# a-rtemis99/hpc_suffix_array

Measured on AMD Instinct MI355X. Metric: suffixes sorted/sec + ms/doubling-round, 1 GiB input at 1/2/4/8 MI355X, higher is better.
Workload: dtype u32

## Files before the change

hpc_suffix_array_amd/_native.py:

```python
from __future__ import annotations

import ctypes
import os
import subprocess

PKG_DIR = os.path.dirname(os.path.abspath(__file__))
LIB_PATH = os.path.join(PKG_DIR, "lib", "libsa_hip.so")
LIB_PATH = os.environ.get("SA_LIB_PATH", LIB_PATH)
CSRC = os.path.join(PKG_DIR, "csrc")

SA_MAX_ROUNDS = 64
KERNEL_KINDS = ["init", "hist_first", "hist_keys", "scan", "scatter_first", "scatter_keys",
                "heads", "heads_scan", "rerank", "seg_count", "seg_scan", "seg_write", "alphabet", "pack",
                "sort_u", "windows", "local_sort", "pivot_keys", "pivot_count", "pivot_write"]
SCHEDULE_PACKED = 0
SCHEDULE_REFERENCE = 1
ROUND1_AUTO = 0
ROUND1_LSD = 1
ROUND1_BUCKETED = 2
SA_K_COUNT = len(KERNEL_KINDS)
FIND_AUTO = 0
FIND_LANE = 1
FIND_WAVE = 2
FIND_LANE_MAX = 3584
FIND_MODES = {"auto": FIND_AUTO, "lane": FIND_LANE, "wave": FIND_WAVE}
BWT_STATS = 258
BWT_TILE = 4096
LOCATE_SA_ORDER = 1
LOCATE_SMALL_CHUNKS = 2
LOCATE_TILE = 2048
LOCATE_ORDERS = {"text": 0, "sa": LOCATE_SA_ORDER}

DROPIN_SYMBOLS = ["create_suffix_array", "destroy_suffix_array", "build_suffix_array",
                  "build_lcp_array", "find_longest_repeated_substring", "is_valid_suffix_array"]
EXT_SYMBOLS = ["sa_context_create", "sa_context_destroy", "sa_context_set_debug", "sa_workspace_bytes", "sa_build_device",
               "sa_build_ex", "sa_check_device", "sa_check", "sa_lcp_device", "sa_lcp", "sa_generate_text_device",
               "sa_alphabet_device", "sa_pack_keys_device", "sa_sort_pairs_device", "sa_scatter_u64_device",
               "sa_gather_u64_device", "sa_running_max_i64_device", "sa_inclusive_sum_i64_device",
               "sa_count_below_u64_device", "sa_select_u8_device",
               "sa_find_device", "sa_find", "sa_find_ex",
               "sa_match_device", "sa_matching_stats_device", "sa_match", "sa_matching_stats",
               "sa_bwt_device", "sa_bwt", "sa_inverse_device", "sa_inverse",
               "sa_locate_device", "sa_locate",
               "sa_dist_begin", "sa_dist_cuts", "sa_dist_plan_cuts", "sa_dist_reserve", "sa_dist_release", "sa_dist_round1", "sa_dist_req_count", "sa_dist_req_fill",
               "sa_dist_answer", "sa_dist_refine",
               "sa_last_error", "sa_host_syncs", "sa_device_count", "sa_version", "sa_struct_size"]


class SAError(RuntimeError):
    """A libsa_hip entry point returned an error code."""


DEBUG_FLAGS = {"no_cmp": 0x1, "no_pk8": 0x2, "no_pad": 0x4, "pad_overflow": 0x8, "no_fast32": 0x10,
               "no_pivot": 0x20, "perm_always": 0x40, "no_xq": 0x80, "xq_overflow": 0x100,
               "no_tied": 0x200, "no_key1_round": 0x400, "no_eonly": 0x800,
               "eonly": 0x1000, "fast32_small": 0x2000, "no_round2_fused": 0x4000,
               "ls_one_wg": 0x8000}


def debug_bits(names) -> int:
    bits = 0
    for x in names or ():
        if x not in DEBUG_FLAGS:
            raise ValueError(f"unknown debug flag {x!r} (one of {sorted(DEBUG_FLAGS)})")
        bits |= DEBUG_FLAGS[x]
    return bits


class SaOpts(ctypes.Structure):
    _fields_ = [("profile", ctypes.c_int32), ("schedule", ctypes.c_int32), ("init_chars", ctypes.c_int32),
                ("radix", ctypes.c_int32), ("round1", ctypes.c_int32), ("debug", ctypes.c_uint32),
                ("span_extra", ctypes.c_int32), ("tune", ctypes.c_int32)]


class SaStats(ctypes.Structure):
    _fields_ = [
        ("rounds", ctypes.c_int32),
        ("n_kinds", ctypes.c_int32),
        ("total_ms", ctypes.c_double),
        ("h2d_ms", ctypes.c_double),
        ("d2h_ms", ctypes.c_double),
        ("round_ms", ctypes.c_double * SA_MAX_ROUNDS),
        ("distinct", ctypes.c_uint64 * SA_MAX_ROUNDS),
        ("passes", ctypes.c_int32 * SA_MAX_ROUNDS),
        ("sorted_n", ctypes.c_uint64 * SA_MAX_ROUNDS),
        ("prefix_len", ctypes.c_uint64 * SA_MAX_ROUNDS),
        ("schedule", ctypes.c_int32),
        ("init_chars", ctypes.c_int32),
        ("sigma", ctypes.c_int32),
        ("sparse_ranks", ctypes.c_int32),
        ("round1", ctypes.c_int32),
        ("largest_window", ctypes.c_int32),
        ("model_bytes", ctypes.c_uint64),
        ("kern_ms", ctypes.c_double * SA_K_COUNT),
        ("kern_launches", ctypes.c_uint64 * SA_K_COUNT),
        ("kern_bytes", ctypes.c_uint64 * SA_K_COUNT),
        ("round1_segments", ctypes.c_int32),
        ("round1_layout", ctypes.c_int32),
        ("round_bytes", ctypes.c_uint64 * SA_MAX_ROUNDS),
        ("round1_windows", ctypes.c_int32 * 4),
    ]

    def to_dict(self) -> dict:
        r = self.rounds
        return {
            "rounds": r,
            "total_ms": self.total_ms,
            "h2d_ms": self.h2d_ms,
            "d2h_ms": self.d2h_ms,
            "round_ms": list(self.round_ms[:r]),
            "distinct": [int(x) for x in self.distinct[:r]],
            "passes": list(self.passes[:r]),
            "sorted_n": [int(x) for x in self.sorted_n[:r]],
            "prefix_len": [int(x) for x in self.prefix_len[:r]],
            "schedule": "reference" if self.schedule == SCHEDULE_REFERENCE else "packed",
            "init_chars": self.init_chars,
            "sigma": self.sigma,
            "sparse_ranks": bool(self.sparse_ranks),
            "round1": {ROUND1_LSD: "lsd", ROUND1_BUCKETED: "bucketed", 3: "pivot"}.get(self.round1, "lsd"),
            "largest_window": self.largest_window,
            "round1_segments": {0: "exact", 1: "padded", 2: "padded-overflow", 3: "striped-records",
                                4: "striped-records-overflow"}.get(self.round1_segments, "exact"),
            "round1_layout": {"compact": bool(self.round1_layout & 1), "pk8": bool(self.round1_layout & 2),
                              "xq": bool(self.round1_layout & 4), "eonly": bool(self.round1_layout & 8)},
            "reference_model_bytes": int(self.model_bytes),
            "round_bytes": [int(x) for x in self.round_bytes[:r]],
            "round1_windows": [int(x) for x in self.round1_windows],
            "kernels": {k: {"ms": self.kern_ms[i], "launches": int(self.kern_launches[i]),
                            "bytes": int(self.kern_bytes[i])} for i, k in enumerate(KERNEL_KINDS)},
        }


DIST_OK = 0
DIST_UNSUPPORTED = 1
DIST_UNBALANCED = 2


class SaDistInfo(ctypes.Structure):
    _fields_ = [("status", ctypes.c_int32), ("sigma", ctypes.c_int32), ("K", ctypes.c_int32),
                ("bucket_bits", ctypes.c_int32), ("m", ctypes.c_uint64), ("sa_off", ctypes.c_uint64),
                ("m_max", ctypes.c_uint64), ("bucket_lo", ctypes.c_uint32), ("bucket_hi", ctypes.c_uint32),
                ("round1_ok", ctypes.c_int32), ("reserved", ctypes.c_int32), ("heads", ctypes.c_uint64),
                ("unsorted", ctypes.c_uint64), ("groups", ctypes.c_uint64)]


class SuffixArrayStruct(ctypes.Structure):
    _fields_ = [("str", ctypes.c_void_p), ("n", ctypes.c_int),
                ("sa", ctypes.POINTER(ctypes.c_int)), ("lcp", ctypes.POINTER(ctypes.c_int))]


_lib = None


def source_hash() -> str:
    import glob
    import hashlib
    h = hashlib.sha256()
    files = sorted(glob.glob(os.path.join(CSRC, "sa_*")) + [os.path.join(CSRC, "Makefile")]
                   + glob.glob(os.path.join(PKG_DIR, "..", "include", "*.h")))
    for p in files:
        with open(p, "rb") as f:
            h.update(os.path.basename(p).encode() + b"\0" + f.read())
    return h.hexdigest()[:16]


def build_library(force: bool = False) -> str:
    if force or not os.path.exists(LIB_PATH):
        subprocess.run(["make", "-s", "-C", CSRC], check=True)
    return LIB_PATH


def lib() -> ctypes.CDLL:
    global _lib
    if _lib is not None:
        return _lib
    if not os.path.exists(LIB_PATH):
        raise SAError(f"{LIB_PATH} is missing: run `make -C {CSRC}` (or __graft_entry__.build())")
    L = ctypes.CDLL(LIB_PATH)
    vp, u64, i32 = ctypes.c_void_p, ctypes.c_uint64, ctypes.c_int
    L.sa_context_create.argtypes = [i32, u64, ctypes.POINTER(vp)]
    L.sa_context_create.restype = i32
    L.sa_context_destroy.argtypes = [vp]
    L.sa_context_destroy.restype = None
    L.sa_context_set_debug.argtypes = [vp, ctypes.POINTER(SaOpts)]
    L.sa_context_set_debug.restype = i32
    L.sa_workspace_bytes.argtypes = [u64]
    L.sa_workspace_bytes.restype = u64
    L.sa_build_device.argtypes = [vp, vp, u64, vp, vp, ctypes.POINTER(SaOpts), ctypes.POINTER(SaStats)]
    L.sa_build_device.restype = i32
    L.sa_build_ex.argtypes = [vp, u64, vp, i32, ctypes.POINTER(SaOpts), ctypes.POINTER(SaStats)]
    L.sa_build_ex.restype = i32
    L.sa_check_device.argtypes = [vp, vp, u64, vp, vp]
    L.sa_check_device.restype = i32
    L.sa_check.argtypes = [vp, u64, vp, i32]
    L.sa_check.restype = i32
    L.sa_lcp_device.argtypes = [vp, vp, u64, vp, vp, ctypes.POINTER(u64), ctypes.POINTER(u64), vp]
    L.sa_lcp_device.restype = i32
    L.sa_lcp.argtypes = [vp, u64, vp, i32, vp, ctypes.POINTER(u64), ctypes.POINTER(u64)]
    L.sa_lcp.restype = i32
    L.sa_alphabet_device.argtypes = [vp, u64, ctypes.POINTER(ctypes.c_uint32), vp]
    L.sa_alphabet_device.restype = i32
    L.sa_pack_keys_device.argtypes = [vp, vp, u64, u64, u64, ctypes.POINTER(ctypes.c_uint16), u64,
                                      ctypes.c_uint32, vp, vp]
    L.sa_pack_keys_device.restype = i32
    L.sa_sort_pairs_device.argtypes = [vp, vp, vp, u64, ctypes.c_uint32, vp, vp, vp]
    L.sa_sort_pairs_device.restype = i32
    L.sa_scatter_u64_device.argtypes = [vp, u64, vp, ctypes.c_int64, vp, u64, vp]
    L.sa_scatter_u64_device.restype = i32
    L.sa_gather_u64_device.argtypes = [vp, vp, u64, vp, ctypes.c_int64, u64, vp]
    L.sa_gather_u64_device.restype = i32
    L.sa_running_max_i64_device.argtypes = [vp, u64, vp]
    L.sa_running_max_i64_device.restype = i32
    L.sa_inclusive_sum_i64_device.argtypes = [vp, u64, vp]
    L.sa_inclusive_sum_i64_device.restype = i32
    L.sa_count_below_u64_device.argtypes = [vp, u64, vp, u64, i32, vp, vp]
    L.sa_count_below_u64_device.restype = i32
    L.sa_select_u8_device.argtypes = [vp, u64, vp, ctypes.POINTER(u64), vp]
    L.sa_select_u8_device.restype = i32
    L.sa_find_device.argtypes = [vp, u64, vp, vp, u64, vp, u64, vp, vp, ctypes.c_uint32, vp]
    L.sa_find_device.restype = i32
    L.sa_find.argtypes = [vp, u64, vp, i32, vp, vp, u64, vp, vp]
    L.sa_find.restype = i32
    L.sa_find_ex.argtypes = [vp, u64, vp, i32, vp, vp, u64, vp, vp, ctypes.c_uint32]
    L.sa_find_ex.restype = i32
    L.sa_match_device.argtypes = [vp, u64, vp, vp, u64, vp, u64, vp, vp, vp, ctypes.c_uint32, vp]
    L.sa_match_device.restype = i32
    L.sa_matching_stats_device.argtypes = [vp, u64, vp, vp, u64, u64, vp, vp, vp, ctypes.c_uint32, vp]
    L.sa_matching_stats_device.restype = i32
    L.sa_match.argtypes = [vp, u64, vp, i32, vp, vp, u64, vp, vp, vp, ctypes.c_uint32]
    L.sa_match.restype = i32
    L.sa_matching_stats.argtypes = [vp, u64, vp, i32, vp, u64, u64, vp, vp, vp, ctypes.c_uint32]
    L.sa_matching_stats.restype = i32
    L.sa_bwt_device.argtypes = [vp, u64, vp, vp, vp, vp]
    L.sa_bwt_device.restype = i32
    L.sa_bwt.argtypes = [vp, u64, vp, i32, vp, vp]
    L.sa_bwt.restype = i32
    L.sa_inverse_device.argtypes = [vp, u64, vp, vp, vp]
    L.sa_inverse_device.restype = i32
    L.sa_inverse.argtypes = [vp, u64, i32, vp]
    L.sa_inverse.restype = i32
    L.sa_locate_device.argtypes = [vp, u64, vp, vp, vp, u64, u64, ctypes.c_uint32, vp, vp, u64, ctypes.POINTER(u64), vp]
    L.sa_locate_device.restype = i32
    L.sa_locate.argtypes = [vp, u64, i32, vp, vp, u64, u64, ctypes.c_uint32, vp, vp, u64]
    L.sa_locate.restype = i32
    DI =ctypes.POINTER(SaDistInfo)
    L.sa_dist_begin.argtypes = [vp, vp, u64, i32, i32, ctypes.POINTER(ctypes.c_uint32), vp, vp, DI]
    L.sa_dist_cuts.argtypes = [vp, ctypes.POINTER(u64), DI]
    L.sa_dist_plan_cuts.argtypes = [i32, u64, i32, ctypes.POINTER(u64), ctypes.POINTER(ctypes.c_uint32),
                                    ctypes.POINTER(u64)]
    L.sa_dist_release.argtypes = [vp]
    L.sa_dist_reserve.argtypes = [vp, u64, i32]
    L.sa_dist_round1.argtypes = [vp, vp, vp, DI, ctypes.POINTER(SaStats)]
    L.sa_dist_req_count.argtypes = [vp, u64, ctypes.POINTER(u64), vp, DI]
    L.sa_dist_req_fill.argtypes = [vp, u64, vp, vp]
    L.sa_dist_answer.argtypes = [vp, vp, u64, vp, vp]
    L.sa_dist_refine.argtypes = [vp, u64, vp, vp, vp, DI]
    for f in (L.sa_dist_begin, L.sa_dist_cuts, L.sa_dist_plan_cuts, L.sa_dist_reserve, L.sa_dist_release,
              L.sa_dist_round1, L.sa_dist_req_count, L.sa_dist_req_fill,
              L.sa_dist_answer, L.sa_dist_refine):
        f.restype = i32
    L.sa_generate_text_device.argtypes = [vp, u64, u64, ctypes.c_char_p, ctypes.c_uint32, vp]
    L.sa_generate_text_device.restype = i32
    L.sa_last_error.argtypes = []
    L.sa_last_error.restype = ctypes.c_char_p
    L.sa_host_syncs.argtypes = []
    L.sa_host_syncs.restype = ctypes.c_uint64
    L.sa_device_count.argtypes = []
    L.sa_device_count.restype = i32
    L.sa_version.argtypes = []
    L.sa_version.restype = ctypes.c_char_p
    P = ctypes.POINTER(SuffixArrayStruct)
    L.create_suffix_array.argtypes = [ctypes.c_char_p, i32]
    L.create_suffix_array.restype = P
    L.destroy_suffix_array.argtypes = [P]
    L.destroy_suffix_array.restype = None
    L.build_suffix_array.argtypes = [P]
    L.build_suffix_array.restype = None
    L.build_lcp_array.argtypes = [P]
    L.build_lcp_array.restype = None
    L.find_longest_repeated_substring.argtypes = [P]
    L.find_longest_repeated_substring.restype = vp
    L.is_valid_suffix_array.argtypes = [P]
    L.is_valid_suffix_array.restype = i32
    _lib = L
    return L


def check(rc: int, what: str) -> int:
    if rc < 0:
        raise SAError(f"{what}: {lib().sa_last_error().decode(errors='replace')} (code {rc})")
    return rc


def device_count() -> int:
    return lib().sa_device_count()


def require_device() -> None:
    if device_count() <= 0:
        raise SAError("no HIP device visible: libsa_hip builds suffix arrays on an MI355X only")
```

hpc_suffix_array_amd/csrc/sa_build.hip:

```cpp
#include <hip/hip_runtime.h>

#include <algorithm>
#include <atomic>
#include <chrono>
#include <cstdarg>
#include <cstdio>
#include <cstdlib>
#include <cstring>
#include <mutex>
#include <string>
#include <thread>
#include <vector>

#include "../../include/sa_hip.h"

#ifndef SA_ALPHA_GRID
#define SA_ALPHA_GRID 2048
#endif

#include "sa_bucket.h"
#include "sa_check.h"
#include "sa_kernels.h"
#include "sa_lcp.h"
#include "sa_limits.h"
// ... 52 lines not shown
#define SA_TRACE(...)                                   \
    do {                                                \
        if (trace_on()) {                               \
            std::fprintf(stderr, "[sa] " __VA_ARGS__);  \
            std::fputc('\n', stderr);                   \
        }                                               \
    } while (0)

#ifndef SA_MAX_CHUNKS
#define SA_MAX_CHUNKS 4096
#endif
constexpr uint32_t kMaxChunks = SA_MAX_CHUNKS;
static_assert(kMaxChunks >= 1 && kMaxChunks <= (1u << 20), "chunk scratch sized for at most 2^20 chunks");
constexpr uint64_t kSparseDiv = 8;
constexpr int kEvPool = 256;
constexpr int kRoundEv = SA_MAX_ROUNDS + 1;
constexpr int kSyncEv = kEvPool + kRoundEv;

static uint64_t align_up(uint64_t x, uint64_t a) { return (x + a - 1) / a * a; }

static uint32_t bit_width(uint64_t x) {
    uint32_t w = 0;
    while (x) { ++w; x >>= 1; }
    return w;
}

static Chunking plan_chunks(uint64_t n) {
    Chunking ch;
    ch.n = n;
    const uint64_t tiles = (n + kTile - 1) / kTile;
    uint64_t tpc = (tiles + kMaxChunks - 1) / kMaxChunks;
    if (tpc == 0) tpc = 1;
    ch.tiles_per_chunk = (uint32_t)tpc;
    ch.chunks = (uint32_t)std::max<uint64_t>(1, (tiles + tpc - 1) / tpc);
    return ch;
}

}

namespace sa { struct DistState; }

struct sa_context {
    int device = 0;
    uint64_t cap = 0;
    uint64_t cap_pad = 0;
    uint64_t ucap = 0;
    uint32_t* rank = nullptr;
    uint64_t* keys[2] = {nullptr, nullptr};
    uint32_t* vals_alt = nullptr;
    uint32_t* vals_u = nullptr;
    uint32_t* u_pos[2] = {nullptr, nullptr};
    uint32_t* u_idx[2] = {nullptr, nullptr};
    uint32_t* u_g[2] = {nullptr, nullptr};
    uint32_t* u_gs[2] = {nullptr, nullptr};
    uint64_t gscap = 0;
    uint64_t* keys_u = nullptr;
    uint64_t kucap = 0;
    uint32_t* segx = nullptr;
    uint64_t segx_words = 0;
    uint32_t* os = nullptr;
    uint32_t* lsd = nullptr;
    uint32_t* lsdx = nullptr;
    uint32_t* segw = nullptr;
    uint64_t* states = nullptr;
    uint32_t epoch = 0;
    int radix = 0;
    int cus = 256;
    uint32_t* member = nullptr;
    uint32_t* hist = nullptr;
    uint32_t* totals = nullptr;
    uint32_t* counts = nullptr;
    uint32_t* words = nullptr;
    uint32_t* alpha = nullptr;
    uint16_t* code = nullptr;
    uint32_t* host_words = nullptr;
    hipEvent_t ev[sa::kEvPool + sa::kRoundEv + 1];
    int ev_ready = 0;
    sa::DistState* dist = nullptr;
    uint32_t dbg = 0;
    int32_t span_extra = 0;
    int32_t tune = 0;
    bool dna = false;
    bool samples_pending = false;
};

namespace sa {

static uint64_t pad_capacity(uint64_t n) { return n + n / 8 + (1ull << 22); }

static uint64_t pad_elems(uint64_t n) {
    const uint64_t m = align_up(std::max<uint64_t>(n, 1), 64);
    return (n >= (1ull << 26) && n <= (1ull << 31)) ? align_up(pad_capacity(n), 64) : m;
}

constexpr uint64_t kMaxRadix = 1024;
static uint64_t tile_states_bytes(uint64_t n) { return ((n + kTile - 1) / kTile + 1) * kMaxRadix * 8; }

static uint64_t ws_bytes(uint64_t n) {
    const uint64_t m = align_up(std::max<uint64_t>(n, 1), 64);
    const uint64_t ku_slack = n >= (1ull << 26) ? n / 16 + 8ull * 1024 * kXqSlack + 64 : 0;
    const uint64_t gs = 2 * (n / 2 + 64) * 4;
    const uint64_t segx = (xq_words(1024) + 1032 + 2ull * kXq * (1ull << 19)) * 4;
    return m * 4 + 2 * m * 8 + m * 4 + (pad_elems(n) - m) * 12 + 7 * m * 4 + (m + ku_slack) * 8 + m / 8 + gs +
           segx + tile_states_bytes(n) + (uint64_t)kRadix * kMaxChunks * 4 + 8192;
}

static void free_ctx_buffers(sa_context* c) {
    hipFree(c->rank);
    hipFree(c->keys[0]);
    hipFree(c->keys[1]);
    hipFree(c->vals_alt);
    hipFree(c->states);
    c->rank = nullptr;
    c->keys[0] = c->keys[1] = nullptr;
    c->vals_alt = nullptr;
    c->states = nullptr;
    c->cap = 0;
    c->cap_pad = 0;
}

static void free_u_buffers(sa_context* c) {
    hipFree(c->vals_u);
    hipFree(c->keys_u);
    hipFree(c->member);
    c->vals_u = nullptr;
    c->keys_u = nullptr;
    c->member = nullptr;
    for (int i = 0; i < 2; ++i) {
        hipFree(c->u_pos[i]);
        hipFree(c->u_idx[i]);
        hipFree(c->u_g[i]);
        hipFree(c->u_gs[i]);
        c->u_pos[i] = c->u_idx[i] = c->u_g[i] = c->u_gs[i] = nullptr;
    }
    c->gscap = 0;
    c->ucap = 0;
    c->kucap = 0;
}

static void set_debug(sa_context* c, const sa_opts* o) {
    c->dbg = o ? o->debug : 0u;
    c->span_extra = o ? o->span_extra : 0;
    c->tune = o ? o->tune : 0;
}

static int ensure_capacity(sa_context* c, uint64_t n) {
    if (n <= c->cap && c->rank) return SA_OK;
    SA_HIP(hipSetDevice(c->device));
    free_ctx_buffers(c);
    const uint64_t m = align_up(std::max<uint64_t>(n, 1), 64);
    const uint64_t mp = pad_elems(n);
    if (hipMalloc(&c->rank, m * 4) != hipSuccess || hipMalloc(&c->keys[0], mp * 8) != hipSuccess ||
        hipMalloc(&c->keys[1], m * 8) != hipSuccess || hipMalloc(&c->vals_alt, mp * 4) != hipSuccess ||
        hipMalloc(&c->states, tile_states_bytes(n)) != hipSuccess ||
        hipMemset(c->states, 0, tile_states_bytes(n)) != hipSuccess) {
        free_ctx_buffers(c);
        (void)hipGetLastError();
        return set_err(SA_E_NOMEM, "device allocation of %.2f GiB workspace failed",
                       (double)ws_bytes(n) / (1ull << 30));
    }
    c->cap = n;
    c->cap_pad = mp;
    SA_TRACE("workspace: rank %p keys0 %p keys1 %p vals_alt %p", (void*)c->rank, (void*)c->keys[0], (void*)c->keys[1],
             (void*)c->vals_alt);
    return SA_OK;
}
// ... 474 lines not shown
            hipLaunchKernelGGL(k_lsd_qbase, dim3(1), dim3(1024), 0, s, (const uint32_t*)qh + p * 8 * kLsdMaxRadix,
                               1u << pl.bits[p], qb);
            tm.end();
            const bool more = p + 1 < pl.P;
            const uint32_t nsh = more ? pl.shift[p + 1] : 0u, nnb = more ? pl.bits[p + 1] : 1u;
            uint32_t* nh = more ? qh + (p + 1) * 8 * kLsdMaxRadix : nullptr;
            uint32_t* tk = qt + p * 8 * 32;
            if (p == 0) {
                tm.begin(SA_K_SCATTER_FIRST);
                SA_TRY(lsd_pass<Src0, PACKED, true>(c, first, n, pl.shift[0], pl.bits[0], qb, tk, kb[0], vb[0], s, nsh,
                                                    nnb, nh, qd, tpq));
                tm.end();
                add_bytes(st, SA_K_SCATTER_FIRST, (8 + pair) * n);
            } else {
                tm.begin(SA_K_SCATTER_KEYS);
                if constexpr (PACKED)
                    SA_TRY(lsd_pass<SrcItems, true, true>(c, SrcItems{kb[(p - 1) & 1]}, n, pl.shift[p], pl.bits[p], qb,
                                                          tk, kb[p & 1], nullptr, s, nsh, nnb, nh, qd, tpq));
                else
                    SA_TRY(lsd_pass<SrcKeys, false, true>(c, SrcKeys{kb[(p - 1) & 1], vb[(p - 1) & 1]}, n, pl.shift[p],
                                                          pl.bits[p], qb, tk, kb[p & 1], vb[p & 1], s, nsh, nnb, nh,
                                                          qd, tpq));
                tm.end();
                add_bytes(st, SA_K_SCATTER_KEYS, 2 * pair * n);
            }
        }
        SA_HIP(hipGetLastError());
        *sorted = kb[(pl.P - 1) & 1];
        return SA_OK;
    }
    tm.begin(SA_K_HIST_FIRST);
    hipLaunchKernelGGL(k_lsd_hist<Src0>, dim3((uint32_t)std::min<uint64_t>((n + 8 * kBlock - 1) / (8 * kBlock),
                                                                           (uint64_t)c->cus * 4)),
                       dim3(kBlock), 0, s, first, n, first_only, lsd_ghist(c));
    tm.end();
    add_bytes(st, SA_K_HIST_FIRST, 8 * n);
    const uint64_t pair = PACKED ? 8 : 12;
    for (uint32_t p = 0; p < pl.P; ++p) {
        uint32_t* base = lsd_base(c) + p * kLsdMaxRadix;
        tm.begin(SA_K_SCAN);
        hipLaunchKernelGGL(k_digit_base_wide, dim3(1), dim3(1024), 0, s,
                           (const uint32_t*)lsd_ghist(c) + p * kLsdMaxRadix, 1u << pl.bits[p], base);
        tm.end();
        const bool more = p + 1 < pl.P;
        const uint32_t nsh = more ? pl.shift[p + 1] : 0u, nnb = more ? pl.bits[p + 1] : 1u;
        uint32_t* nh = more ? lsd_ghist(c) + (p + 1) * kLsdMaxRadix : nullptr;
        if (p == 0) {
            tm.begin(SA_K_SCATTER_FIRST);
            SA_TRY(lsd_pass<Src0, PACKED>(c, first, n, pl.shift[0], pl.bits[0], base, lsd_tickets(c), kb[0], vb[0], s,
                                          nsh, nnb, nh));
            tm.end();
            add_bytes(st, SA_K_SCATTER_FIRST, (8 + pair) * n);
        } else {
            tm.begin(SA_K_SCATTER_KEYS);
            if constexpr (PACKED)
                SA_TRY(lsd_pass<SrcItems, true>(c, SrcItems{kb[(p - 1) & 1]}, n, pl.shift[p], pl.bits[p], base,
                                                lsd_tickets(c) + p, kb[p & 1], nullptr, s, nsh, nnb, nh));
            else
                SA_TRY(lsd_pass<SrcKeys, false>(c, SrcKeys{kb[(p - 1) & 1], vb[(p - 1) & 1]}, n, pl.shift[p],
                                                pl.bits[p], base, lsd_tickets(c) + p, kb[p & 1], vb[p & 1], s, nsh,
                                                nnb, nh));
            tm.end();
            add_bytes(st, SA_K_SCATTER_KEYS, 2 * pair * n);
        }
    }
    SA_HIP(hipGetLastError());
    *sorted = kb[(pl.P - 1) & 1];
    return SA_OK;
}

#ifndef SA_INIT_HIST
#define SA_INIT_HIST 1
#endif
static int build_reference(sa_context* c, const uint8_t* d_text, uint64_t n, uint32_t* d_sa, hipStream_t s,
                           sa_stats* st, Timer& tm) {
    int rc = SA_OK;
    const Chunking ch = plan_chunks(n);
    uint32_t* h_alpha = c->host_words + 64;
    uint16_t* h_code = reinterpret_cast<uint16_t*>(c->host_words + 320);
    SA_HIP(hipMemsetAsync(c->alpha, 0, 8 * 4, s));
    tm.begin(SA_K_ALPHABET);
    {
        const uint32_t grid = (uint32_t)std::min<uint64_t>((n + kBlock * 16 - 1) / (kBlock * 16), SA_ALPHA_GRID);
        hipLaunchKernelGGL(k_alphabet, dim3(grid), dim3(kBlock), 0, s, d_text, n, c->alpha);
    }
    tm.end();
    add_bytes(st, SA_K_ALPHABET, n);
    SA_HIP(hipMemcpyAsync(h_alpha, c->alpha, 8 * 4, hipMemcpyDeviceToHost, s));
    SA_HIP(host_sync(s));
    uint32_t sigma = 0;
    for (int b = 0; b < 256; ++b) h_code[b] = ((h_alpha[b >> 5] >> (b & 31)) & 1u) ? (uint16_t)(++sigma) : 0;
    SA_HIP(hipMemcpyAsync(c->code, h_code, 256 * 2, hipMemcpyHostToDevice, s));
    uint64_t D = sigma;
    const uint64_t perm_min = perm_min_n(c);
    const uint32_t ib = std::max<uint32_t>(1, bit_width(n - 1));
    bool used_perm = false;
    bool hist_ready = false;
    tm.begin(SA_K_INIT);
    {
        const uint32_t w1 = bit_width(D);
        const bool packed1 = c->radix == 0 && 2 * w1 + ib <= 64;
        const LsdPlan pl1 = lsd_plan(2 * w1, packed1 ? ib : 0, lsd_max_bits(c));
        if (SA_INIT_HIST && c->radix == 0 && lsd_xq_ok(c, n, pl1, packed1)) {
            uint32_t tpq;
            uint64_t qspan;
            QDiv qd;
            lsd_xq_span(n, &tpq, &qspan, &qd);
            SA_HIP(hipMemsetAsync(c->lsdx, 0, 8 * kLsdMaxRadix * 4, s));
            const uint64_t grid = std::min<uint64_t>((n + kBlock * 16 - 1) / (kBlock * 16), 4ull * (uint64_t)c->cus);
            hipLaunchKernelGGL(k_init_rank_hist, dim3((uint32_t)grid), dim3(kBlock), 0, s, d_text, n,
                               (const uint16_t*)c->code, c->rank, w1, pl1.shift[0] - (packed1 ? ib : 0u),
                               (1u << pl1.bits[0]) - 1u, qd, c->lsdx);
            hist_ready = true;
        } else {
            const uint64_t grid = std::min<uint64_t>((n + kBlock * 4 - 1) / (kBlock * 4), 4096);
            hipLaunchKernelGGL(k_init_rank_dense, dim3((uint32_t)grid), dim3(kBlock), 0, s, d_text, n,
                               (const uint16_t*)c->code, c->rank);
        }
    }
    tm.end();
    SA_HIP(hipGetLastError());
    add_bytes(st, SA_K_INIT, 5 * n);
    if (st) st->sigma = (int32_t)sigma;

    tm.round_mark();
    for (uint64_t h = 1;; h *= 2) {
        const uint32_t w = bit_width(D);
        const bool packed = c->radix == 0 && 2 * w + ib <= 64;
        SA_TRACE("reference round h=%llu D=%llu w=%u%s", (unsigned long long)h, (unsigned long long)D, w,
                 packed ? " packed" : "");
        SrcRank src{c->rank, n, h, w};
        uint64_t* sorted;
        uint32_t P;
        if (c->radix == 0) {
            const LsdPlan pl = lsd_plan(2 * w, packed ? ib : 0, lsd_max_bits(c));
            P = pl.P;
            rc = packed ? lsd_sort<true>(c, SrcRankPk{c->rank, n, h, w, ib}, n, pl, d_sa, c->vals_alt, s, tm, st,
                                         &sorted, hist_ready)
                        : lsd_sort<false>(c, src, n, pl, d_sa, c->vals_alt, s, tm, st, &sorted, hist_ready);
        } else {
            rc = radix_sort(c, src, 4 * n, ch, 2 * w, d_sa, c->vals_alt, c->keys[0], c->keys[1], s, tm, st, &sorted,
                            &P);
        }
        if (rc) return rc;
        const bool use_perm = packed || n >= perm_min;
        const uint32_t ptiles = (uint32_t)((n + kPermTile - 1) / kPermTile);
        tm.begin(SA_K_HEADS);
        if (use_perm)
            hipLaunchKernelGGL((k_tile_heads<kPermBlock, kPermItems>), dim3(ptiles), dim3(kPermBlock), 0, s,
                               (const uint64_t*)sorted, n, packed ? ib : 0u, perm_tile_off(c));
        else
            hipLaunchKernelGGL(k_heads, dim3(ch.chunks), dim3(kBlock), 0, s, sorted, ch, c->counts, 0u);
        tm.end();
        tm.begin(SA_K_HEADS_SCAN);
        if (use_perm)
            hipLaunchKernelGGL(k_scan_heads, dim3(1), dim3(kBlock), 0, s, perm_tile_off(c), ptiles, c->words);
        else
            hipLaunchKernelGGL(k_scan_heads, dim3(1), dim3(kBlock), 0, s, c->counts, ch.chunks, c->words);
        tm.end();
        SA_HIP(hipGetLastError());
        add_bytes(st, SA_K_HEADS, 8 * n);
        add_bytes(st, SA_K_HEADS_SCAN, 8ull * ch.chunks);
        SA_HIP(hipMemcpyAsync(c->host_words, c->words, 4 * (kPermErrWord + 1), hipMemcpyDeviceToHost, s));
        SA_HIP(host_sync(s));
        if (c->host_words[4]) return set_err(SA_E_INTERNAL, "radix look-back did not complete");
        if (used_perm && c->host_words[kPermErrWord])
            return set_err(SA_E_INTERNAL, "re-rank permutation lost a suffix (flags %u)", c->host_words[kPermErrWord]);
// ... 290 lines not shown
    *sorted = ukb0;
    return SA_OK;
}

static int pivot_round1(sa_context* c, uint64_t n, uint32_t bits1, uint32_t* d_sa, hipStream_t s, Timer& tm,
                        sa_stats* st, bool* done, uint64_t* D, uint64_t* m, uint64_t* G, uint32_t* P) {
    *done = false;
    const Chunking ch = plan_chunks(n);
    const uint64_t* keys = c->keys[1];
    uint32_t* const gs = c->u_pos[1];
    uint32_t* const toff = gs + 2;
    uint32_t* const tid = gs + 4;
    uint32_t* const gP = c->vals_alt;
    uint32_t* const cc = c->hist;
    c->host_words[24] = 0;
    c->host_words[25] = (uint32_t)n;
    SA_HIP(hipMemcpyAsync(gs, c->host_words + 24, 8, hipMemcpyHostToDevice, s));
    tm.begin(SA_K_PIVOT_COUNT);
    hipLaunchKernelGGL((k_pivot_pass<0, true>), dim3(ch.chunks), dim3(kBlock), 0, s, keys, nullptr, nullptr, ch,
                       (const uint32_t*)gs, nullptr, 1u, 0u, cc, gP, nullptr, nullptr, nullptr, nullptr, TiedOut{});
    hipLaunchKernelGGL(k_scan_rows, dim3(3), dim3(kBlock), 0, s, cc, ch.chunks, c->totals);
    tm.end();
    SA_HIP(hipGetLastError());
    add_bytes(st, SA_K_PIVOT_COUNT, 8 * n);
    SA_HIP(hipMemcpyAsync(c->host_words + 16, c->totals, 12, hipMemcpyDeviceToHost, s));
    SA_HIP(host_sync(s));
    const uint64_t t0 = c->host_words[16], t1 = c->host_words[17], t2 = c->host_words[18];
    if (t0 + t1 + t2 != n) return set_err(SA_E_INTERNAL, "round-1 pivot classes %llu + %llu + %llu != %llu",
                                          (unsigned long long)t0, (unsigned long long)t1, (unsigned long long)t2,
                                          (unsigned long long)n);
    SA_TRACE("  round 1: pivot split, tied %llu of %llu", (unsigned long long)t1, (unsigned long long)n);
    if (t1 * 2 < n) return SA_OK;
    const uint64_t mr = t0 + t2;
    uint64_t* const rk = c->keys[0];
    uint32_t* const ridx = c->u_idx[1];
    if (!gs_available(c, n)) return SA_OK;
    tm.begin(SA_K_PIVOT_WRITE);
    hipLaunchKernelGGL(k_pivot_gp, dim3(1), dim3(kBlock), 0, s, (const uint32_t*)gs, 1u, (const uint32_t*)cc, ch,
                       (const uint32_t*)c->totals, gP);
    hipLaunchKernelGGL(k_pivot_tied_scan, dim3(1), dim3(kBlock), 0, s, (const uint32_t*)gP, 1u, toff, tid,
                       c->totals + 4);
    const TiedOut to{nullptr, toff, tid, c->rank, d_sa, c->u_pos[0], c->u_idx[0], c->u_g[0], c->u_gs[0]};
    hipLaunchKernelGGL((k_pivot_pass<3, true>), dim3(ch.chunks), dim3(kBlock), 0, s, keys, nullptr, nullptr, ch,
                       (const uint32_t*)gs, nullptr, 1u, 0u, cc, gP, nullptr, nullptr, rk, ridx, to);
    tm.end();
    SA_HIP(hipGetLastError());
    add_bytes(st, SA_K_PIVOT_WRITE, 8 * n + 16 * t1 + 12 * mr);
    SA_HIP(hipMemcpyAsync(c->host_words + 20, c->totals + 4, 12, hipMemcpyDeviceToHost, s));
    SA_HIP(host_sync(s));
    const uint64_t T = c->host_words[20], Gt = c->host_words[21], Dt = c->host_words[22];
    if (T > t1 || Gt > 1 || Dt > 1)
        return set_err(SA_E_INTERNAL, "round-1 tied block %llu / %llu / %llu out of range", (unsigned long long)T,
                       (unsigned long long)Gt, (unsigned long long)Dt);
    uint32_t Pr = 0;
    uint64_t Dr = 0, mrr = 0, Gr = 0;
    if (mr > 0) {
        const uint32_t Pn = (bits1 + 7) / 8;
        uint32_t* const vfinal = (Pn & 1u) ? c->u_g[1] : ridx;
        uint32_t* const vother = (Pn & 1u) ? ridx : c->u_g[1];
        uint64_t* rs = nullptr;
        int rc = radix_sort(c, SrcKeys{rk, ridx}, 12 * mr, plan_chunks(mr), bits1, vfinal, vother, c->keys_u, rk, s,
                            tm, st, &rs, &Pr);
        if (rc) return rc;
        rc = segments(c, rs, vfinal, plan_chunks(mr), PosGap{t0, t1}, false, nullptr, d_sa, 0, s, tm, st, &Dr, &mrr,
                      &Gr, nullptr, 0, RankMap{}, T, (uint32_t)Gt, c->u_gs[0]);
        if (rc) return rc;
    }
    *done = true;
    *D = Dr + Dt;
    *m = mrr + T;
    *G = Gr + Gt;
    *P = 2 + Pr;
    return SA_OK;
}

static int build_packed(sa_context* c, const uint8_t* d_text, uint64_t n, uint32_t* d_sa, hipStream_t s,
                        const sa_opts* opts, sa_stats* st, Timer& tm) {
    int rc = SA_OK;
    rc = ensure_u_capacity(c, n);
    if (rc) return rc;
    tm.round_mark();
    uint32_t* h_alpha = c->host_words + 64;
    uint16_t* h_code = reinterpret_cast<uint16_t*>(c->host_words + 320);
    SA_HIP(hipMemsetAsync(c->alpha, 0, 8 * 4, s));
    tm.begin(SA_K_ALPHABET);
    {
        const uint32_t grid = (uint32_t)std::min<uint64_t>((n + kBlock * 16 - 1) / (kBlock * 16), SA_ALPHA_GRID);
        hipLaunchKernelGGL(k_alphabet, dim3(grid), dim3(kBlock), 0, s, d_text, n, c->alpha);
    }
    tm.end();
    SA_HIP(hipGetLastError());
    add_bytes(st, SA_K_ALPHABET, n);
    SA_HIP(hipMemcpyAsync(h_alpha, c->alpha, 8 * 4, hipMemcpyDeviceToHost, s));
    const uint32_t tail_n = (uint32_t)std::min<uint64_t>(n, (uint64_t)kMaxK);
    uint8_t* h_tail = reinterpret_cast<uint8_t*>(c->host_words + 2048);
    SA_HIP(hipMemcpyAsync(h_tail, d_text + (n - tail_n), tail_n, hipMemcpyDeviceToHost, s));
    SA_HIP(host_sync(s));
    uint32_t sigma = 0;
    for (int b = 0; b < 256; ++b) h_code[b] = ((h_alpha[b >> 5] >> (b & 31)) & 1u) ? (uint16_t)(++sigma) : 0;
    SA_HIP(hipMemcpyAsync(c->code, h_code, 256 * 2, hipMemcpyHostToDevice, s));
    c->dna = sigma == 4 && h_code['A'] && h_code['C'] && h_code['G'] && h_code['T'];
    uint32_t K = choose_chars(sigma, n, opts ? opts->init_chars : 0);
    const uint64_t base = (uint64_t)sigma + 1;
    const Chunking ch = plan_chunks(n);
    uint64_t* keys1 = nullptr;
    uint32_t ksh1 = 0;
    c->samples_pending = false;
    uint32_t P = 0;

    BucketPlan bp;
    const int r1 = opts ? opts->round1 : SA_ROUND1_AUTO;
    const uint32_t Kb = (opts && opts->init_chars > 0) || sigma <= 1 ? K : min_chars(sigma, n);
    bool bucketed = plan_bucketed(sigma, n, Kb, r1, c->radix, &bp, 1, (c->dbg & SA_DEBUG_NO_CMP) ? 0 : 1);
    if (bucketed && bp.bs.cmp && short_suffix_ties(h_tail, n, tail_n, h_code, sigma, bp.bs.s, bp.bs.R))
        bucketed = plan_bucketed(sigma, n, Kb, r1, c->radix, &bp, 1, 0);
    const bool force_eonly = (c->dbg & SA_DEBUG_EONLY) != 0;
    if (bucketed && bp.bs.cmp == 1 && ((sigma & (sigma - 1)) != 0 || force_eonly) && !(c->dbg & SA_DEBUG_NO_EONLY)) {
        const uint32_t hb = bp.bs.bb - kLoBits;
        BucketPlan b2;
        if ((force_eonly || !plan_pk8(bp, hb, c->dbg, true)) && plan_bucketed(sigma, n, Kb, r1, c->radix, &b2, 1, 2) &&
            (force_eonly || plan_pk8(b2, hb, c->dbg, true)) &&
            !short_suffix_ties(h_tail, n, tail_n, h_code, sigma, b2.bs.s, b2.bs.R, b2.K))
            bp = b2;
    }
    bool fused = false;
    bool r1_pivot = false;
    uint64_t D = 0, m = 0, G = 0;
    uint64_t seg1[3] = {0, 0, 0};
    int r2 = 0;
    if (bucketed) {
        bool done = false;
        rc = round1_bucketed(c, d_text, n, d_sa, bp, full_range(bp, n), s, tm, st, &done, &fused, seg1, &ksh1, true,
                             true, &r2);
        if (rc) return rc;
        bucketed = done;
        if (done) {
            keys1 = c->keys[0];
            P = 2;
            K = bp.K;
        }
    }
    if (!bucketed) {
        const uint32_t bits1 = key_bits(base, K);
        SA_TRACE("packed: sigma=%u K=%u bits=%u", sigma, K, bits1);
        uint64_t top = 1;
        for (uint32_t t = 1; t < K; ++t) top *= base;
        if (c->radix == 0) {
            rc = onesweep_prepare(c, s);
            if (rc) return rc;
        }
        tm.begin(SA_K_PACK);
        hipLaunchKernelGGL(k_pack_text, dim3(ch.chunks), dim3(kBlock), 0, s, d_text, n, (const uint16_t*)c->code, ch,
                           base, top, K, c->keys[1], c->hist, c->radix == 0 ? (bits1 + 7) / 8 : 0u, os_ghist(c));
        tm.end();
        SA_HIP(hipGetLastError());
        add_bytes(st, SA_K_PACK, 9 * n);
        if (c->radix == 0 && !(c->dbg & SA_DEBUG_NO_PIVOT) && n >= (1u << 16)) {
            rc = pivot_round1(c, n, bits1, d_sa, s, tm, st, &r1_pivot, &D, &m, &G, &P);
            if (rc) return rc;
        }
        if (!r1_pivot) {
            SrcKeysIota src{c->keys[1]};
            rc = radix_sort(c, src, 8 * n, ch, bits1, d_sa, c->vals_alt, c->keys[0], c->keys[1], s, tm, st, &keys1,
                            &P, true);
            if (rc) return rc;
        }
    }
    if (st) {
        st->init_chars = (int32_t)K;
        st->sigma = (int32_t)sigma;
        st->round1 = bucketed ? SA_ROUND1_BUCKETED : r1_pivot ? SA_ROUND1_PIVOT : SA_ROUND1_LSD;
    }
    int uo = 0;
    bool sparse = false;
    bool gs_ok[2] = {false, false};
    if (r1_pivot) {
        gs_ok[0] = true;
    } else if (bucketed && fused) {
        D = seg1[0];
        m = seg1[1];
        G = seg1[2];
        sparse = true;
    } else {
        rc = segments(c, keys1, d_sa, ch, PosIdentity{}, true, &sparse, nullptr, uo, s, tm, st, &D, &m, &G, nullptr,
                      0, RankMap{}, 0, 0, gs_buf(c, n, uo));
        if (rc) return rc;
        gs_ok[uo] = gs_buf(c, n, uo) != nullptr;
    }
    uint64_t* ukb0 = keys1 == c->keys[0] ? c->keys[1] : c->keys[0];
    uint64_t* ukb1 = c->keys_u;
    const RankLookup rl{c->rank, c->member, keys1, d_text, (const uint16_t*)c->code, n, base, K,
                        bucketed ? 1u : 0u, bp.bs, bucketed ? c->segw + kBstartOff : nullptr, d_sa, ksh1};
    if (st) st->sparse_ranks = sparse ? 1 : 0;
    auto ensure_samples = [&]() -> int {
        if (!c->samples_pending) return SA_OK;
        c->samples_pending = false;
        const uint64_t ns = (n + (1ull << ksh1) - 1) >> ksh1;
        const uint32_t g = (uint32_t)std::max<uint64_t>(1, std::min<uint64_t>((ns + kBlock - 1) / kBlock, 8192));
        tm.begin(SA_K_SORT_U);
        hipLaunchKernelGGL(k_key1_samples, dim3(g), dim3(kBlock), 0, s, d_text, n, (const uint16_t*)c->code, bp.bs,
                           (const uint32_t*)d_sa, ksh1, keys1);
        tm.end();
        SA_HIP(hipGetLastError());
        add_bytes(st, SA_K_SORT_U, 12 * ns);
        return SA_OK;
    };
    if (r2 == 0) tm.round_mark();
    record_round(st, 0.f, D, P, n, K);
    SA_TRACE("  round 1: D=%llu unsorted=%llu groups=%llu", (unsigned long long)D, (unsigned long long)m,
             (unsigned long long)G);
    if (r2 == 2) {
        tm.round_mark();
        D = n;
        record_round(st, 0.f, D, 1, m, 2 * (uint64_t)K);
        SA_TRACE("  round h=%u: sorted %llu from the local sort's staging, D=%llu", K, (unsigned long long)m,
                 (unsigned long long)D);
        m = 0;
        G = 0;
    }

    const uint32_t wr = bit_width(n);
    for (uint64_t h = K; m > 0; h *= 2) {
        if (h >= 2 * n) return set_err(SA_E_INTERNAL, "doubling did not converge (h=%llu)", (unsigned long long)h);
        const uint32_t wg = G > 1 ? bit_width(G - 1) : 0;
// ... 931 lines not shown
    for (int j = 0; j < kRmItems; ++j) bits |= (b0 + j < m && mask[b0 + j]) ? 1u << j : 0u;
    int64_t o = toff[blockIdx.x] + rm_block_excl<ScanSum>((int64_t)__popc(bits), s_w);
    while (bits) {
        const int j = __builtin_ctz(bits);
        bits &= bits - 1u;
        out[o++] = (int64_t)(b0 + j);
    }
}

template <class Op>
static int scan_i64(int64_t* d_v, uint64_t m, hipStream_t s) {
    const uint64_t tiles = (m + kRmTile - 1) / kRmTile;
    if (tiles > 0xFFFFFFFFull) return set_err(SA_E_INVALID, "m too large");
    int64_t* d_t = nullptr;
    SA_HIP(hipMallocAsync((void**)&d_t, (tiles + 1) * 8, s));
    hipLaunchKernelGGL(k_rmax_tiles<Op>, dim3((uint32_t)tiles), dim3(kRmBlock), 0, s, d_v, m, d_t);
    hipLaunchKernelGGL(k_rmax_carry<Op>, dim3(1), dim3(kRmBlock), 0, s, d_t, tiles);
    hipLaunchKernelGGL(k_rmax_apply<Op>, dim3((uint32_t)tiles), dim3(kRmBlock), 0, s, d_v, m, d_t);
    SA_HIP(hipGetLastError());
    SA_HIP(hipFreeAsync(d_t, s));
    return SA_OK;
}

#include "sa_locate.h"

extern "C" {

int sa_running_max_i64_device(int64_t* d_v, uint64_t m, void* stream) {
    if (m == 0) return SA_OK;
    if (!d_v) return set_err(SA_E_INVALID, "NULL device pointer");
    return scan_i64<ScanMax>(d_v, m, (hipStream_t)stream);
}

int sa_inclusive_sum_i64_device(int64_t* d_v, uint64_t m, void* stream) {
    if (m == 0) return SA_OK;
    if (!d_v) return set_err(SA_E_INVALID, "NULL device pointer");
    return scan_i64<ScanSum>(d_v, m, (hipStream_t)stream);
}

int sa_count_below_u64_device(const uint64_t* d_sorted, uint64_t m, const uint64_t* d_q, uint64_t nq, int right,
                              int64_t* d_out, void* stream) {
    if (nq == 0) return SA_OK;
    if ((!d_sorted && m) || !d_q || !d_out) return set_err(SA_E_INVALID, "NULL device pointer");
    hipStream_t s = (hipStream_t)stream;
    const uint32_t grid = (uint32_t)std::min<uint64_t>((nq + kBlock - 1) / kBlock, 8192);
    if (right) hipLaunchKernelGGL(k_count_below<true>, dim3(grid), dim3(kBlock), 0, s, d_sorted, m, d_q, nq, d_out);
    else hipLaunchKernelGGL(k_count_below<false>, dim3(grid), dim3(kBlock), 0, s, d_sorted, m, d_q, nq, d_out);
    SA_HIP(hipGetLastError());
    return SA_OK;
}

int sa_select_u8_device(const uint8_t* d_mask, uint64_t m, int64_t* d_out, uint64_t* count, void* stream) {
    if (!count) return set_err(SA_E_INVALID, "count is NULL");
    *count = 0;
    if (m == 0) return SA_OK;
    if (!d_mask) return set_err(SA_E_INVALID, "NULL device pointer");
    hipStream_t s = (hipStream_t)stream;
    const uint64_t tiles = (m + kRmTile - 1) / kRmTile;
    if (tiles > 0xFFFFFFFFull) return set_err(SA_E_INVALID, "m too large");
    int64_t* d_t = nullptr;
    int64_t total = 0;
    SA_HIP(hipMallocAsync((void**)&d_t, (tiles + 1) * 8, s));
    hipLaunchKernelGGL(k_sel_count, dim3((uint32_t)tiles), dim3(kRmBlock), 0, s, d_mask, m, d_t);
    hipLaunchKernelGGL(k_rmax_carry<ScanSum>, dim3(1), dim3(kRmBlock), 0, s, d_t, tiles);
    if (d_out) hipLaunchKernelGGL(k_sel_write, dim3((uint32_t)tiles), dim3(kRmBlock), 0, s, d_mask, m, d_t, d_out);
    SA_HIP(hipGetLastError());
    SA_HIP(hipMemcpyAsync(&total, d_t + tiles, 8, hipMemcpyDeviceToHost, s));
    SA_HIP(hipFreeAsync(d_t, s));
    SA_HIP(host_sync(s));
    *count = (uint64_t)total;
    return SA_OK;
}

int sa_alphabet_device(const uint8_t* d_text, uint64_t n, uint32_t present_out[8], void* stream) {
    if (!present_out) return set_err(SA_E_INVALID, "present_out is NULL");
    std::memset(present_out, 0, 32);
    if (n == 0) return SA_OK;
    if (!d_text) return set_err(SA_E_INVALID, "NULL device pointer");
    hipStream_t s = (hipStream_t)stream;
    uint32_t* d_mask = nullptr;
    SA_HIP(hipMallocAsync((void**)&d_mask, 32, s));
    SA_HIP(hipMemsetAsync(d_mask, 0, 32, s));
    const uint32_t grid = (uint32_t)std::min<uint64_t>((n + kBlock * 16 - 1) / (kBlock * 16), 2048);
    hipLaunchKernelGGL(k_alphabet, dim3(grid), dim3(kBlock), 0, s, d_text, n, d_mask);
    SA_HIP(hipGetLastError());
    SA_HIP(hipMemcpyAsync(present_out, d_mask, 32, hipMemcpyDeviceToHost, s));
    SA_HIP(hipFreeAsync(d_mask, s));
    SA_HIP(host_sync(s));
    return SA_OK;
}

int sa_pack_keys_device(sa_context* ctx, const uint8_t* d_text, uint64_t n, uint64_t lo, uint64_t hi,
                        const uint16_t code[256], uint64_t base, uint32_t K, uint64_t* d_keys_out, void* stream) {
    if (lo > hi || hi > n) return set_err(SA_E_INVALID, "bad range [%llu, %llu) of %llu", (unsigned long long)lo,
                                          (unsigned long long)hi, (unsigned long long)n);
    if (K == 0 || K >= (uint32_t)kMaxK || base < 2 || key_bits(base, K) > 64)
        return set_err(SA_E_INVALID, "bad packing K=%u base=%llu", K, (unsigned long long)base);
    if (hi == lo) return SA_OK;
    if (!ctx || !d_text || !d_keys_out || !code) return set_err(SA_E_INVALID, "NULL argument");
    hipStream_t s = (hipStream_t)stream;
    SA_HIP(hipSetDevice(ctx->device));
    uint16_t* h_code = reinterpret_cast<uint16_t*>(ctx->host_words + 320);
    std::memcpy(h_code, code, 512);
    SA_HIP(hipMemcpyAsync(ctx->code, h_code, 512, hipMemcpyHostToDevice, s));
    SA_HIP(host_sync(s));
    uint64_t top = 1;
    for (uint32_t t = 1; t < K; ++t) top *= base;
    const Chunking ch = plan_chunks(hi - lo);
    hipLaunchKernelGGL(k_pack_text, dim3(ch.chunks), dim3(kBlock), 0, s, d_text + lo, n - lo,
                       (const uint16_t*)ctx->code, ch, base, top, K, d_keys_out, (uint32_t*)nullptr, 0u,
                       (uint32_t*)nullptr);
    SA_HIP(hipGetLastError());
    return SA_OK;
}

int sa_sort_pairs_device(sa_context* ctx, const uint64_t* d_keys_in, const uint32_t* d_vals_in, uint64_t m,
                         uint32_t bits, uint64_t* d_keys_out, uint32_t* d_vals_out, void* stream) {
    if (!ctx || !d_keys_in || !d_vals_in || !d_keys_out || !d_vals_out) return set_err(SA_E_INVALID, "NULL argument");
    if (bits == 0 || bits > 64) return set_err(SA_E_INVALID, "bits must be 1..64");
    if (m == 0) return SA_OK;
    if (m > 0xFFFFFFFFull) return set_err(SA_E_INVALID, "m too large");
    if ((const void*)d_keys_in == (const void*)d_keys_out || (const void*)d_vals_in == (const void*)d_vals_out)
        return set_err(SA_E_INVALID, "outputs may not alias inputs");
    hipStream_t s = (hipStream_t)stream;
    SA_HIP(hipSetDevice(ctx->device));
    int rc = ensure_capacity(ctx, m);
    if (rc) return rc;
    ctx->radix = 0;
    SA_HIP(hipMemsetAsync(ctx->words, 0, 64, s));
    Timer tm{ctx, s, false, nullptr};
    const Chunking ch = plan_chunks(m);
    SrcKeys src{d_keys_in, d_vals_in};
    uint64_t* sorted;
    uint32_t P;
    rc = radix_sort(ctx, src, 12 * m, ch, bits, d_vals_out, ctx->vals_alt, d_keys_out, ctx->keys[1], s, tm, nullptr,
                    &sorted, &P);
    if (rc) return rc;
    if (sorted != d_keys_out) SA_HIP(hipMemcpyAsync(d_keys_out, sorted, m * 8, hipMemcpyDeviceToDevice, s));
    SA_HIP(hipMemcpyAsync(ctx->host_words, ctx->words, 20, hipMemcpyDeviceToHost, s));
    SA_HIP(host_sync(s));
    if (ctx->host_words[4]) return set_err(SA_E_INTERNAL, "radix look-back did not complete");
    return SA_OK;
}

int sa_generate_text_device(uint8_t* d_out, uint64_t n, uint64_t seed, const uint8_t* alphabet, uint32_t sigma,
                            void* stream) {
    if (n == 0) return SA_OK;
    if (!d_out || !alphabet || sigma == 0 || sigma > 256) return set_err(SA_E_INVALID, "bad generator arguments");
    Alphabet a;
    std::memset(a.sym, 0, sizeof a.sym);
    std::memcpy(a.sym, alphabet, sigma);
    const uint32_t grid = (uint32_t)std::min<uint64_t>((n + kBlock - 1) / kBlock, 16384);
    hipLaunchKernelGGL(k_gen_text, dim3(grid), dim3(kBlock), 0, (hipStream_t)stream, d_out, n, seed, a, sigma);
    SA_HIP(hipGetLastError());
    return SA_OK;
}

int sa_dist_begin(sa_context* ctx, const uint8_t* d_text, uint64_t n, int world, int rank,
                  const uint32_t present[8], uint64_t* d_coarse, void* stream, sa_dist_info* info) {
    if (!ctx || !info) return set_err(SA_E_INVALID, "NULL argument");
    return dist_begin(ctx, d_text, n, world, rank, present, d_coarse, (hipStream_t)stream, info);
}

int sa_dist_cuts(sa_context* ctx, const uint64_t* h_coarse, sa_dist_info* info) {
    if (!ctx || !info) return set_err(SA_E_INVALID, "NULL argument");
    return dist_cuts(ctx, h_coarse, info);
}
// ... 92 lines not shown
```

hpc_suffix_array_amd/csrc/sa_dropin.cpp:

```cpp
#include <cstddef>
#include <cstdint>
#include <cstdio>
#include <cstdlib>
#include <cstring>
#include <vector>

#include "../../include/sa_hip.h"
#include "../../include/suffix_array.h"

static_assert(sizeof(SuffixArray) == 32, "SuffixArray must keep the reference's 32-byte layout");
static_assert(offsetof(SuffixArray, n) == 8 && offsetof(SuffixArray, sa) == 16 && offsetof(SuffixArray, lcp) == 24,
              "SuffixArray field offsets must match suffix_array.h:16-21");

[[noreturn]] static void die(const char* what) {
    std::fprintf(stderr, "libsa_hip: %s failed: %s\n", what, sa_last_error());
    std::abort();
}

extern "C" {

SuffixArray* create_suffix_array(const char* S, int n) {
    if (n < 0) return nullptr;
    SuffixArray* sa = (SuffixArray*)std::malloc(sizeof(SuffixArray));
    if (!sa) return nullptr;
    sa->n = n;
    sa->str = (char*)std::malloc((size_t)n + 1);
    if (!sa->str) {
        std::free(sa);
        return nullptr;
    }
    std::strncpy(sa->str, S ? S : "", (size_t)n);
    sa->str[n] = '\0';
    sa->sa = (int*)std::malloc((size_t)(n ? n : 1) * sizeof(int));
    sa->lcp = (int*)std::malloc((size_t)(n ? n : 1) * sizeof(int));
    if (!sa->sa || !sa->lcp) {
        std::free(sa->str);
        std::free(sa->sa);
        std::free(sa->lcp);
        std::free(sa);
        return nullptr;
    }
    return sa;
}

void destroy_suffix_array(SuffixArray* sa) {
    if (!sa) return;
    std::free(sa->str);
    std::free(sa->sa);
    std::free(sa->lcp);
    std::free(sa);
}

void build_suffix_array(SuffixArray* sa) {
    if (!sa || sa->n <= 0) return;
    if (sa_build_ex((const uint8_t*)sa->str, (uint64_t)sa->n, sa->sa, 4, nullptr, nullptr) != SA_OK)
        die("build_suffix_array");
}

void build_lcp_array(SuffixArray* sa) {
    if (!sa || sa->n <= 0) return;
    if (sa_lcp((const uint8_t*)sa->str, (uint64_t)sa->n, sa->sa, 4, sa->lcp, nullptr, nullptr) != SA_OK)
        die("build_lcp_array");
}

char* find_longest_repeated_substring(SuffixArray* sa) {
    if (!sa || !sa->lcp) return nullptr;
    int best = 0, at = -1;
    for (int r = 1; r < sa->n; ++r)
        if (sa->lcp[r] > best) {
            best = sa->lcp[r];
            at = r;
        }
    if (best == 0) return nullptr;
    char* out = (char*)std::malloc((size_t)best + 1);
    if (!out) return nullptr;
    std::strncpy(out, sa->str + sa->sa[at], (size_t)best);
    out[best] = '\0';
    return out;
}

int is_valid_suffix_array(SuffixArray* sa) {
    if (!sa || sa->n <= 0) return 1;
    const int r = sa_check((const uint8_t*)sa->str, (uint64_t)sa->n, sa->sa, 4);
    if (r < 0) die("is_valid_suffix_array");
    return r;
}

}

extern "C" uint64_t sa_struct_size(int which) {
    return which == 0 ? sizeof(sa_stats) : which == 1 ? sizeof(sa_opts) : 0;
}
```

hpc_suffix_array_amd/csrc/sa_kernels.h:

```cpp
#pragma once
#include <hip/hip_runtime.h>
#include <stdint.h>

#include "sa_search.h"

namespace sa {

constexpr int kWave = 64;
constexpr int kBlock = 256;
constexpr int kWaves = kBlock / kWave;
constexpr int kItems = 16;
constexpr int kTile = kBlock * kItems;
constexpr int kWaveTile = kWave * kItems;
constexpr int kRadix = 256;

__device__ __forceinline__ uint32_t lane_id() { return threadIdx.x & (kWave - 1); }
__device__ __forceinline__ uint32_t wave_id() { return threadIdx.x / kWave; }
__device__ __forceinline__ uint64_t lanemask_lt() { return (1ull << lane_id()) - 1ull; }

struct SrcRank {
    const uint32_t* __restrict__ rank;
    uint64_t n;
    uint64_t h;
    uint32_t w;
    __device__ __forceinline__ uint64_t key(uint64_t e) const {
        const uint64_t r0 = rank[e];
        const uint64_t r1 = (e + h < n) ? rank[e + h] : 0u;
        return (r0 << w) | r1;
    }
    __device__ __forceinline__ uint32_t val(uint64_t e) const { return (uint32_t)e; }
    static constexpr bool kRaw = true;
    __device__ __forceinline__ uint64_t raw(uint64_t e) const {
        return (uint64_t)rank[e] | ((uint64_t)((e + h < n) ? rank[e + h] : 0u) << 32);
    }
    __device__ __forceinline__ uint64_t finish(uint64_t r, uint64_t) const {
        return ((r & 0xFFFFFFFFull) << w) | (r >> 32);
    }
};

struct SrcText {
    const uint8_t* __restrict__ text;
    const uint16_t* __restrict__ code;
    uint64_t n;
    uint64_t base;
    uint32_t K;
    __device__ __forceinline__ uint64_t key(uint64_t e) const {
        uint64_t x = 0;
        if (e + K <= n) {
            for (uint32_t t = 0; t < K; ++t) x = x * base + code[text[e + t]];
        } else {
            for (uint32_t t = 0; t < K; ++t) x = x * base + ((e + t < n) ? code[text[e + t]] : 0u);
        }
        return x;
    }
    __device__ __forceinline__ uint32_t val(uint64_t e) const { return (uint32_t)e; }
};

struct BucketSpec {
    uint64_t pow_s1;
    uint64_t powR1;
    uint64_t cmul;
    uint32_t sigma, s, R, rb;
    uint32_t bb, bsh;
    uint32_t cmp;
};

__host__ __device__ __forceinline__ uint64_t bucket_low(const BucketSpec& b, uint64_t r, uint64_t L) {
    if (b.cmp == 2) return r;
    if (b.cmp) return 2 * r + (L >= b.s + b.R ? 1u : 0u);
    if (L < b.s) return L - 1;
    const uint64_t tl = L - b.s < b.R ? L - b.s : b.R;
    return b.s + r * (b.R + 1) + tl;
}

struct CodeMap {
    const uint16_t* __restrict__ code;
    __device__ __forceinline__ uint32_t operator[](uint32_t b) const {
        const uint32_t c = code[b];
        return c ? c - 1u : 0u;
    }
};

constexpr int kKeyWords = 8;

template <bool FULL, class Map>
__device__ __forceinline__ uint64_t key1_words(const uint8_t* __restrict__ text, uint64_t n, const Map& s_map,
// ... 494 lines not shown
            bool ok;
            const uint64_t m = wave_heads(keys, w0 + (uint64_t)j * kWave, e1, prev_last, key, ok, kshift);
            cnt += (uint32_t)__popcll(m);
        }
    }
    uint32_t tot;
    block_exclusive_sum(lane_id() == 0 ? cnt : 0u, s_tmp, &tot);
    if (threadIdx.x == 0) counts[c] = tot;
}

__global__ __launch_bounds__(kBlock) void k_scan_heads(uint32_t* __restrict__ counts, uint32_t chunks,
                                                       uint32_t* __restrict__ d_total) {
    __shared__ uint32_t s_tmp[kWaves];
    uint32_t carry = 0;
    for (uint32_t base = 0; base < chunks; base += kBlock * 4) {
        uint32_t v[4], sum = 0;
#pragma unroll
        for (int j = 0; j < 4; ++j) {
            const uint32_t i = base + threadIdx.x * 4 + j;
            v[j] = (i < chunks) ? counts[i] : 0u;
            sum += v[j];
        }
        uint32_t tot;
        uint32_t off = block_exclusive_sum(sum, s_tmp, &tot) + carry;
#pragma unroll
        for (int j = 0; j < 4; ++j) {
            const uint32_t i = base + threadIdx.x * 4 + j;
            if (i < chunks) counts[i] = off;
            off += v[j];
        }
        carry += tot;
    }
    if (threadIdx.x == 0) *d_total = carry;
}

__global__ __launch_bounds__(kBlock) void k_rerank(const uint64_t* __restrict__ keys,
                                                   const uint32_t* __restrict__ idx, Chunking ch,
                                                   const uint32_t* __restrict__ chunk_off,
                                                   uint32_t* __restrict__ rank) {
    __shared__ uint32_t s_wtot[kWaves];
    __shared__ uint32_t s_tmp[kWaves];
    const uint32_t c = blockIdx.x;
    const uint64_t e0 = ch.begin(c), e1 = ch.end(c);
    uint32_t run = chunk_off[c];
    for (uint64_t tb = e0; tb < e1; tb += kTile) {
        const uint64_t w0 = tb + (uint64_t)wave_id() * kWaveTile;
        uint64_t prev_last = (w0 > 0 && w0 < e1) ? keys[w0 - 1] : 0ull;
        uint64_t m[kItems];
        uint32_t wsum = 0;
#pragma unroll
        for (int j = 0; j < kItems; ++j) {
            uint64_t key;
            bool ok;
            m[j] = wave_heads(keys, w0 + (uint64_t)j * kWave, e1, prev_last, key, ok);
            wsum += (uint32_t)__popcll(m[j]);
        }
        if (lane_id() == 0) s_wtot[wave_id()] = wsum;
        __syncthreads();
        uint32_t woff = run, ttot = 0;
#pragma unroll
        for (int w = 0; w < kWaves; ++w) {
            const uint32_t x = s_wtot[w];
            woff += (w < (int)wave_id()) ? x : 0u;
            ttot += x;
        }
        __syncthreads();
        const uint64_t le_mask = lanemask_lt() | (1ull << lane_id());
#pragma unroll
        for (int j = 0; j < kItems; ++j) {
            const uint64_t e = w0 + (uint64_t)j * kWave + lane_id();
            if (e < e1) {
                const uint32_t x = idx[e];
                if (x < ch.n) rank[x] = woff + (uint32_t)__popcll(m[j] & le_mask);
            }
            woff += (uint32_t)__popcll(m[j]);
        }
        run += ttot;
    }
    (void)s_tmp;
}


__global__ __launch_bounds__(kBlock) void k_alphabet(const uint8_t* __restrict__ text, uint64_t n,
                                                     uint32_t* __restrict__ present) {
    __shared__ uint32_t s_m[kBlock * 9];
    uint32_t* m = s_m + threadIdx.x * 9;
#pragma unroll
    for (int i = 0; i < 8; ++i) m[i] = 0;
    auto add = [&](uint32_t b) { atomicOr(&m[b >> 5], 1u << (b & 31u)); };
    const uint64_t stride = (uint64_t)gridDim.x * kBlock * 16;
    auto whole = [&](uint64_t i) { return i + 16 <= n && (((uintptr_t)(text + i)) & 15) == 0; };
    uint64_t i = ((uint64_t)blockIdx.x * kBlock + threadIdx.x) * 16;
    uint4 v = make_uint4(0u, 0u, 0u, 0u);
    if (i < n && whole(i)) v = *reinterpret_cast<const uint4*>(text + i);
    uint32_t step = 0;
    for (; i < n; i += stride) {
        if (step && (step & (step - 1)) == 0) {
            uint32_t all = ~0u;
#pragma unroll
            for (int q = 0; q < 8; ++q) {
                uint32_t x = m[q];
#pragma unroll
                for (int o = 32; o >= 1; o >>= 1) x |= __shfl_xor(x, o, kWave);
                all &= x;
            }
            if (all == ~0u) break;
        }
        ++step;
        const uint64_t in = i + stride;
        uint4 vn = make_uint4(0u, 0u, 0u, 0u);
        if (in < n && whole(in)) vn = *reinterpret_cast<const uint4*>(text + in);
        if (whole(i)) {
            const uint32_t w4[4] = {v.x, v.y, v.z, v.w};
            uint32_t o = v.x | v.y | v.z | v.w, a = v.x & v.y & v.z & v.w;
            o |= o >> 16;
            o |= o >> 8;
            a &= a >> 16;
            a &= a >> 8;
            if (((o ^ a) & 0xE0u) == 0u) {
                uint32_t bits = 0;
#pragma unroll
                for (int q = 0; q < 4; ++q)
#pragma unroll
                    for (int b = 0; b < 4; ++b) bits |= 1u << ((w4[q] >> (8 * b)) & 31u);
                atomicOr(&m[(o & 0xFFu) >> 5], bits);
            } else {
#pragma unroll
                for (int q = 0; q < 4; ++q)
#pragma unroll
                    for (int b = 0; b < 4; ++b) add((w4[q] >> (8 * b)) & 0xFFu);
            }
        } else {
            for (uint64_t j = i; j < n && j < i + 16; ++j) add(text[j]);
        }
        v = vn;
    }
    __shared__ uint32_t s_or[8];
    if (threadIdx.x < 8) s_or[threadIdx.x] = 0;
    __syncthreads();
#pragma unroll
    for (int i = 0; i < 8; ++i) {
        uint32_t x = m[i];
#pragma unroll
        for (int o = 32; o >= 1; o >>= 1) x |= __shfl_xor(x, o, kWave);
        if (lane_id() == 0 && x) atomicOr(&s_or[i], x);
    }
    __syncthreads();
    if (threadIdx.x < 8) {
        const uint32_t x = s_or[threadIdx.x];
        if (x & ~__hip_atomic_load(&present[threadIdx.x], __ATOMIC_RELAXED, __HIP_MEMORY_SCOPE_AGENT))
            atomicOr(&present[threadIdx.x], x);
    }
}

__device__ __forceinline__ void hist_add_runs_valid(uint32_t (*s_h)[kRadix], uint64_t k, bool valid, uint32_t p_lo,
                                                    uint32_t p_hi, uint32_t row0) {
    const uint32_t lane = lane_id();
    const uint64_t above = lane == 63 ? 0ull : (~0ull << (lane + 1));
    for (uint32_t p = p_lo; p < p_hi; ++p) {
        const uint32_t d = valid ? ((uint32_t)(k >> (8 * p)) & 0xFFu) : 0x100u;
        const uint32_t dl = __shfl_up(d, 1, 64);
        const bool head = lane == 0 || dl != d;
        const uint64_t hm = __ballot(head) & above;
        const uint32_t next = hm ? (uint32_t)__ffsll((long long)hm) - 1u : 64u;
        if (head && valid) atomicAdd(&s_h[row0 + p][d], next - lane);
    }
}

constexpr int kPackRun = kTile / kBlock;
constexpr int kMaxK = 64;
constexpr int kPackMaxPasses = 8;

__global__ __launch_bounds__(kBlock) void k_pack_text(const uint8_t* __restrict__ text, uint64_t avail,
                                                      const uint16_t* __restrict__ code, Chunking ch,
                                                      uint64_t base, uint64_t top, uint32_t K,
                                                      uint64_t* __restrict__ keys, uint32_t* __restrict__ hist,
                                                      uint32_t passes, uint32_t* __restrict__ ghist) {
    __shared__ uint16_t s_code[256];
    __shared__ uint16_t s_c[kTile + kMaxK];
    __shared__ uint32_t s_hist[kPackMaxPasses][kRadix];
    __shared__ uint64_t s_k[kTile + kTile / kPackRun];
    s_code[threadIdx.x] = code[threadIdx.x];
    for (int i = threadIdx.x; i < kPackMaxPasses * kRadix; i += kBlock) (&s_hist[0][0])[i] = 0;
    const uint32_t c = blockIdx.x;
    const uint64_t e0 = ch.begin(c), e1 = ch.end(c);
    const uint64_t n = avail;
    auto count = [&](uint64_t key, bool valid) {
        if (passes == 0) hist_add_runs_valid(s_hist, key, valid, 0, 1, wave_id());
        else hist_add_runs_valid(s_hist, key, valid, 0, passes, 0);
    };
    __syncthreads();
    for (uint64_t tb = e0; tb < e1; tb += kTile) {
        {
            const uint64_t i = tb + (uint64_t)threadIdx.x * 16;
            uint16_t* dst = s_c + threadIdx.x * 16;
            if (i + 16 <= n && (((uintptr_t)(text + i)) & 15) == 0) {
                const uint4 v = *reinterpret_cast<const uint4*>(text + i);
                const uint32_t w4[4] = {v.x, v.y, v.z, v.w};
#pragma unroll
                for (int q = 0; q < 4; ++q)
#pragma unroll
                    for (int b = 0; b < 4; ++b) dst[4 * q + b] = s_code[(w4[q] >> (8 * b)) & 0xFFu];
            } else {
                for (int q = 0; q < 16; ++q) dst[q] = (i + q < n) ? s_code[text[i + q]] : (uint16_t)0;
            }
            if (threadIdx.x < K) {
                const uint64_t h = tb + kTile + threadIdx.x;
                s_c[kTile + threadIdx.x] = (h < n) ? s_code[text[h]] : (uint16_t)0;
            }
        }
        __syncthreads();
        const uint32_t l0 = threadIdx.x * kPackRun;
        uint64_t x = 0;
        for (uint32_t t = 0; t < K; ++t) x = x * base + s_c[l0 + t];
        uint64_t* kd = s_k + threadIdx.x * (kPackRun + 1);
        kd[0] = x;
        count(x, tb + l0 < e1);
#pragma unroll
        for (int j = 1; j < kPackRun; ++j) {
            x = (x - (uint64_t)s_c[l0 + j - 1] * top) * base + s_c[l0 + j - 1 + K];
            kd[j] = x;
            count(x, tb + l0 + j < e1);
        }
        __syncthreads();
#pragma unroll
        for (int j = 0; j < kPackRun; ++j) {
            const uint32_t q = j * kBlock + threadIdx.x;
            const uint64_t g = tb + q;
            if (g < e1) keys[g] = s_k[q + q / kPackRun];
        }
        __syncthreads();
    }
    if (passes == 0) {
        uint32_t s = 0;
#pragma unroll
        for (int w = 0; w < kWaves; ++w) s += s_hist[w][threadIdx.x];
        if (hist) hist[(uint64_t)threadIdx.x * ch.chunks + c] = s;
    } else {
        for (uint32_t p = 0; p < passes; ++p) {
            const uint32_t v = s_hist[p][threadIdx.x];
            if (v) atomicAdd(&ghist[p * kRadix + threadIdx.x], v);
        }
    }
}

struct PosIdentity {
    __device__ __forceinline__ uint32_t operator()(uint64_t s) const { return (uint32_t)s; }
};
struct PosArray {
    const uint32_t* __restrict__ p;
    __device__ __forceinline__ uint32_t operator()(uint64_t s) const { return p[s]; }
};
struct PosGap {
// ... 290 lines not shown
```

hpc_suffix_array_amd/csrc/sa_limits.h:

```cpp
#pragma once
#include <cstdint>

namespace sa {

constexpr uint32_t kXqQueues = 8;
constexpr uint32_t kXqRegionSlack = 2048;
constexpr uint32_t kXqMaxDigits = 1024;

constexpr uint64_t xq_region_space(uint64_t m) {
    return m + m / 16 + (uint64_t)kXqQueues * kXqMaxDigits * kXqRegionSlack;
}

constexpr bool xq_offsets_fit(uint64_t m) { return xq_region_space(m) <= 0xFFFFFFFFull; }

}
```

hpc_suffix_array_amd/csrc/sa_round1.h:

```cpp
#pragma once

#ifndef SA_HIST_WPC
#define SA_HIST_WPC 64
#endif
#ifndef SA_REC_STRIPED
#define SA_REC_STRIPED 1
#endif
#ifndef SA_BB_EXTRA
#define SA_BB_EXTRA 0
#endif
#ifndef SA_ITEMS_A
#define SA_ITEMS_A 12
#endif
#ifndef SA_TEXT_BLOCK
#define SA_TEXT_BLOCK 512
#endif
#ifndef SA_LIST_BLOCK
#define SA_LIST_BLOCK 1024
#endif


#ifndef SA_SEG_BLOCK
#define SA_SEG_BLOCK 1024
#endif
#ifndef SA_SEG_XQ
#define SA_SEG_XQ 1
#endif
#ifndef SA_ITEMS_B
#define SA_ITEMS_B 10
#endif
#ifndef SA_ITEMS_PK
#define SA_ITEMS_PK 12
#endif
#ifndef SA_KEY_SAMPLE
#define SA_KEY_SAMPLE 4
#endif
constexpr uint32_t kKeySample = SA_KEY_SAMPLE;
#ifndef SA_LAZY_SAMPLES
#define SA_LAZY_SAMPLES 1
#endif
constexpr uint64_t kPadMinN = 1ull << 26;
#ifndef SA_LS_VARIANT
#define SA_LS_VARIANT 0
#endif
static int ls_variant(const sa_context* c) {
    const uint32_t t = ((uint32_t)c->tune >> 16) & 0xFu;
    return t ? (int)(t - 1u) : SA_LS_VARIANT;
}

static uint32_t text_stripes(const sa_context* c) {
    const uint32_t e = ((uint32_t)c->tune >> 8) & 0xFFu;
    const uint32_t v = e ? e : 8u;
    return v >= 8 ? 8u : v >= 4 ? 4u : v >= 2 ? 2u : 1u;
}

__global__ __launch_bounds__(kLoRadix) void k_sum_rows(const uint32_t* __restrict__ in, uint32_t rows,
                                                       uint32_t* __restrict__ out) {
    uint32_t t = 0;
    for (uint32_t r = 0; r < rows; ++r) t += in[r * kLoRadix + threadIdx.x];
    out[threadIdx.x] = t;
}
constexpr uint64_t kPadMaxN = 1ull << 31;
constexpr int kUsFlagWord = 12;

static uint32_t key1_bits(const BucketSpec& bs) {
    unsigned __int128 dmax = 1;
    for (uint32_t t = 0; t < bs.s; ++t) dmax *= bs.sigma;
    const unsigned __int128 kmax = ((dmax - 1) << bs.rb) | (((unsigned __int128)1 << bs.rb) - 1);
    uint32_t kw = 0;
    for (unsigned __int128 x = kmax + 1; x; x >>= 1) ++kw;
    return kw;
}
constexpr uint32_t kPadStartOff = kLoRadix + 1024;
constexpr uint32_t kPadDenseOff = kPadStartOff + kLoRadix + 64;

struct BucketPlan {
    BucketSpec bs{};
    uint32_t ib = 0;
    uint32_t K = 0;
};

static bool plan_bucketed(uint32_t sigma, uint64_t n, uint32_t K, int round1, int radix, BucketPlan* p,
                          int world = 1, int cmp = 0) {
    if (round1 == SA_ROUND1_LSD || radix != 0 || sigma < 2 || n < 2) return false;
    if (round1 == SA_ROUND1_AUTO && n < kBucketMinN) return false;
    uint32_t bb = std::max<uint32_t>(16u, bit_width(n - 1) > 13 ? bit_width(n - 1) - 13 : 0u);
    if (world <= 1) bb = std::min<uint32_t>(bb, 18u);
    bb += SA_BB_EXTRA;
    if (bb > 18 + (uint32_t)bit_width((uint64_t)std::max(world, 1) - 1) || bb > 24) return false;
    uint64_t ps = 1;
    uint32_t s = 0;
    while (ps < (1ull << bb)) {
        ps *= sigma;
        ++s;
    }
    while (ps % (1ull << bb) != 0 && ps < (64ull << bb) && s + 1 < K && ps * sigma <= (1ull << 32)) {
        ps *= sigma;
        ++s;
    }
    if (ps > (1ull << 32)) return false;
    if (K <= s || K > (uint32_t)kMaxK) return false;
    const uint32_t ib = bit_width(n - 1);
    const uint32_t bd = bit_width(ps - 1);
    const uint32_t span = bit_width((ps + (1ull << bb) - 1) >> bb) + 1;
    for (uint32_t R = K - s; R >= 1; --R) {
        unsigned __int128 pr = 1;
        for (uint32_t t = 0; t < R; ++t) pr *= sigma;
        unsigned __int128 lowmax = cmp == 2 ? pr - 1 : cmp ? 2 * pr - 1 : s + (pr - 1) * (R + 1) + R;
        uint32_t rb = 0;
        while (lowmax) {
            ++rb;
            lowmax >>= 1;
        }
        if (bd + rb > 64 || rb + span + ib > 64) continue;
        p->bs.pow_s1 = ps / sigma;
        p->bs.powR1 = (uint64_t)(pr / sigma);
        p->bs.cmul = (1ull << 48) / ps;
        p->bs.bb = bb;
        p->bs.bsh = 48u - bb;
        p->bs.sigma = sigma;
        p->bs.s = s;
        p->bs.R = R;
        p->bs.rb = rb;
        p->bs.cmp = (uint32_t)cmp;
        p->ib = ib;
        p->K = s + R;
        return true;
    }
    return false;
}

static bool short_suffix_ties(const uint8_t* tail, uint64_t n, uint32_t t, const uint16_t* code, uint32_t sigma,
                              uint32_t s, uint32_t R, uint32_t last = 0) {
    auto dig = [&](uint8_t x) -> uint32_t { return code[x] ? code[x] - 1u : 0u; };
    const uint32_t K = s + R;
    if (last == 0) last = K - 1;
    uint64_t Ds[kMaxK + 1];
    unsigned __int128 rs[kMaxK + 1];
    uint32_t cnt = 0;
    for (uint32_t L = 1; L <= last && L <= n && L <= t; ++L) {
        const uint8_t* x = tail + (t - L);
        uint64_t D = 0;
        unsigned __int128 r = 0;
        for (uint32_t q = 0; q < s; ++q) D = D * sigma + (q < L ? dig(x[q]) : 0u);
        for (uint32_t q = s; q < K; ++q) r = r * sigma + (q < L ? dig(x[q]) : 0u);
        for (uint32_t o = 0; o < cnt; ++o)
            if (Ds[o] == D && rs[o] == r) return true;
        Ds[cnt] = D;
        rs[cnt] = r;
        ++cnt;
    }
    return false;
}

static bool plan_pk8(const BucketPlan& bp, uint32_t hb, uint32_t dbg, bool np2 = false) {
    const uint32_t sg = bp.bs.sigma;
    if (sg < 2 || (dbg & SA_DEBUG_NO_PK8)) return false;
    if ((sg & (sg - 1)) != 0) {
        if (!np2) return false;
        const uint64_t ps = bp.bs.pow_s1 * sg;
        const uint64_t per = ((ps + (1ull << bp.bs.bb) - 1) >> bp.bs.bb) + 1;
        return hb + bit_width(per - 1) + bp.bs.rb + bp.ib <= 64;
    }
    const uint32_t lg = (uint32_t)__builtin_ctz(sg);
    if (lg * bp.bs.s < bp.bs.bb) return false;
    return hb + (lg * bp.bs.s - bp.bs.bb) + bp.bs.rb + bp.ib <= 64;
}

struct BucketRange {
    uint32_t blo = 0, bhi = 0;
    uint64_t m = 0;
    uint64_t sa_off = 0;
    bool always_u = false;
    uint32_t* rank = nullptr;
    uint32_t* member = nullptr;
    uint32_t* prefix = nullptr;
    uint32_t* tmp_rank = nullptr;
};

static BucketRange full_range(const BucketPlan& bp, uint64_t n) {
    BucketRange r;
    r.blo = 0;
    r.bhi = 1u << bp.bs.bb;
    r.m = n;
    return r;
}

static uint32_t range_hb(uint32_t nb) {
    const uint32_t w = bit_width(nb > 1 ? nb - 1 : 1);
    return std::max<uint32_t>(7u, w > kLoBits ? w - kLoBits : 0u);
}

static int round1_bucketed(sa_context* c, const uint8_t* d_text, uint64_t n, uint32_t* d_sa, const BucketPlan& bp,
                           const BucketRange& br_, hipStream_t s, Timer& tm, sa_stats* st, bool* done, bool* fused,
                           uint64_t seg[3], uint32_t* ksh, bool allow_pad = true, bool allow_xq = true,
                           int* round2 = nullptr) {
    *done = false;
    *fused = false;
    *ksh = 0;
    if (round2) *round2 = 0;
    const uint64_t m = br_.m;
    const uint32_t blo = br_.blo, bhi = br_.bhi;
    if (bhi <= blo || bhi - blo > (1u << 18)) return set_err(SA_E_INTERNAL, "bucket range [%u, %u)", blo, bhi);
    int rc = onesweep_prepare(c, s);
    if (rc) return rc;
    SA_HIP(hipMemsetAsync(c->words, 0, 12, s));
    SA_HIP(hipMemsetAsync(c->words + 5, 0, 28, s));
    const bool listed = m * 10 <= n * 3;
    uint64_t* const lkeys = c->keys_u;
    uint32_t* const lpos = c->vals_u;
    const uint64_t rtiles = (n + kTile - 1) / kTile;
    const uint32_t rgrid = (uint32_t)(std::min<uint64_t>(rtiles, (uint64_t)SA_HIST_WPC * (uint32_t)c->cus) /
                                      kRecStripes * kRecStripes);
    const uint64_t rcap64 = (c->dbg & SA_DEBUG_PAD_OVERFLOW) ? m / kRecStripes / 2 + 1
                                                             : (m + m / 8) / kRecStripes + 2 * (uint64_t)kTile;
    const bool striped = SA_REC_STRIPED && listed && allow_pad && !(c->dbg & SA_DEBUG_NO_PAD) &&
                         rtiles >= 4ull * kRecStripes && rgrid >= kRecStripes && kRecStripes * rcap64 <= c->ucap;
    const uint32_t rcap = (uint32_t)std::min<uint64_t>(rcap64, UINT32_MAX);
    uint32_t* const rcur = c->hist;
    const bool padded = allow_pad && !listed && blo == 0 && bhi == (1u << bp.bs.bb) && n >= kPadMinN &&
                        n <= kPadMaxN && c->cap_pad >= pad_capacity(n) && !(c->dbg & SA_DEBUG_NO_PAD);
    const uint32_t ssh = std::max<uint32_t>(6u, bit_width(n) > 21 ? bit_width(n) - 21 : 0u);
    uint32_t* const pstart = os_base(c) + kPadStartOff;
    uint32_t* const dlo = os_base(c) + kPadDenseOff;
    if (st) st->round1_segments = padded ? 1 : striped ? 3 : 0;
    tm.begin(SA_K_PACK);
    if (padded) {
        const bool pow2 = (bp.bs.sigma & (bp.bs.sigma - 1)) == 0;
        const uint32_t g = (uint32_t)std::max<uint64_t>(1, std::min<uint64_t>(((n >> ssh) + kBlock - 1) / kBlock,
                                                                               4u * (uint32_t)c->cus));
        if (pow2)
            hipLaunchKernelGGL(k_bucket_sample<true>, dim3(g), dim3(kBlock), 0, s, d_text, n,
                               (const uint16_t*)c->code, bp.bs, ssh, os_ghist(c));
        else
            hipLaunchKernelGGL(k_bucket_sample<false>, dim3(g), dim3(kBlock), 0, s, d_text, n,
                               (const uint16_t*)c->code, bp.bs, ssh, os_ghist(c));
        hipLaunchKernelGGL(k_pad_starts, dim3(1), dim3(kLoRadix), 0, s, (const uint32_t*)os_ghist(c), ssh,
                           (c->dbg & SA_DEBUG_PAD_OVERFLOW) ? 1u : 0u, (uint32_t)c->cap_pad, pstart);
    } else {
        const uint64_t tiles = (n + kTile - 1) / kTile;
        const uint32_t g = (uint32_t)std::max<uint64_t>(1, std::min<uint64_t>(tiles, (uint64_t)SA_HIST_WPC * (uint32_t)c->cus));
        const bool pow2 = (bp.bs.sigma & (bp.bs.sigma - 1)) == 0;
        uint32_t* const wgcnt = c->hist;
        uint32_t* const wgoff = c->hist + g;
#define SA_HIST_G(G, P, L, W)                                                                                 \
    hipLaunchKernelGGL((k_bucket_hist<P, false, L>), dim3(G), dim3(kBlock), 0, s, d_text, n,                  \
                       (const uint16_t*)c->code, bp.bs, os_ghist(c), 0ull, n, blo, bhi, lkeys, lpos, W, rcap,  \
                       c->words + 11)
#define SA_HIST_ID_G(G, L, W)                                                                                 \
    hipLaunchKernelGGL((k_bucket_hist<true, false, L, true>), dim3(G), dim3(kBlock), 0, s, d_text, n,         \
                       (const uint16_t*)c->code, bp.bs, os_ghist(c), 0ull, n, blo, bhi, lkeys, lpos, W, rcap,  \
                       c->words + 11)
#define SA_HIST(P, L, W) SA_HIST_G(g, P, L, W)
#define SA_HIST_ID(L, W) SA_HIST_ID_G(g, L, W)
        const bool ident = bp.bs.sigma == 256;
        if (striped) {
            SA_HIP(hipMemsetAsync(rcur, 0, kRecStripes * kRecCurStride * 4, s));
            if (ident) SA_HIST_ID_G(rgrid, 3, rcur);
            else if (pow2 && SA_DNA_SWAR && c->dna)
                hipLaunchKernelGGL((k_bucket_hist<true, false, 3, false, true>), dim3(rgrid), dim3(kBlock), 0, s, d_text,
                                   n, (const uint16_t*)c->code, bp.bs, os_ghist(c), 0ull, n, blo, bhi, lkeys, lpos, rcur,
                                   rcap, c->words + 11);
            else if (pow2) SA_HIST_G(rgrid, true, 3, rcur);
            else SA_HIST_G(rgrid, false, 3, rcur);
            SA_HIP(hipMemcpyAsync(c->host_words + 11, c->words + 11, 4, hipMemcpyDeviceToHost, s));
            SA_HIP(host_sync(s));
            if (c->host_words[11]) {
                SA_TRACE("  bucketed round 1: a record stripe overflowed, again with the counting scan");
                tm.end();
                const int rc = round1_bucketed(c, d_text, n, d_sa, bp, br_, s, tm, st, done, fused, seg, ksh, false,
                                               allow_xq, round2);
                if (st) st->round1_segments = 4;
                return rc;
            }
        } else if (ident && listed) SA_HIST_ID(1, wgcnt);
        else if (pow2 && listed) SA_HIST(true, 1, wgcnt);
        else if (pow2) SA_HIST(true, 0, wgcnt);
        else if (listed) SA_HIST(false, 1, wgcnt);
        else SA_HIST(false, 0, wgcnt);
        if (listed && !striped) {
            hipLaunchKernelGGL(k_exscan_u32, dim3(1), dim3(kBlock), 0, s, (const uint32_t*)wgcnt, wgoff, g);
            if (ident) SA_HIST_ID(2, wgoff);
            else if (pow2) SA_HIST(true, 2, wgoff);
            else SA_HIST(false, 2, wgoff);
        }
#undef SA_HIST
#undef SA_HIST_ID
#undef SA_HIST_G
#undef SA_HIST_ID_G
    }
    tm.end();
    add_bytes(st, SA_K_PACK, padded ? (n >> ssh) * 64 : n + (striped ? 12 * m : listed ? n + 12 * m : 0));
    const uint32_t hb = (blo == 0 && bhi == (1u << bp.bs.bb)) ? bp.bs.bb - kLoBits : range_hb(bhi - blo);
    if (hb < 7 || hb > 10) return set_err(SA_E_INTERNAL, "second bucket pass of %u bits", hb);
    const uint32_t nb_tab = 1u << (hb + kLoBits);
    const bool np2 = (bp.bs.sigma & (bp.bs.sigma - 1)) != 0;
    const bool pk8 = plan_pk8(bp, hb, c->dbg, !br_.always_u);
    uint32_t bits1 = 0;
    if (bp.bs.cmp) {
        const uint64_t ps = bp.bs.pow_s1 * bp.bs.sigma, per = (ps + (1ull << bp.bs.bb) - 1) >> bp.bs.bb;
        const bool exact = (ps & ((1ull << bp.bs.bb) - 1)) == 0;
        bits1 = bit_width(exact ? per - 1 : per) + bp.bs.rb;
        if (c->span_extra > 0) bits1 = std::min<uint32_t>(bits1 + (uint32_t)c->span_extra, 64u - bp.ib);
    }
    const bool fast32 = bits1 > (uint32_t)kSubBits && bits1 - kSubBits <= kLowMax &&
                        (m / (uint64_t)(bhi - blo) >= 4ull * kWinStride || (c->dbg & SA_DEBUG_FAST32_SMALL)) &&
                        !(c->dbg & SA_DEBUG_NO_FAST32);
    static_assert(kXqQueues == kXq && kXqRegionSlack == kXqSlack, "sa_limits.h mirrors sa_split.h");
    const bool xq = SA_SEG_XQ && allow_xq && fast32 && c->cus % (int)kXq == 0 && !(c->dbg & SA_DEBUG_NO_XQ) &&
                    c->kucap >= xq_region_space(m) + kWave && xq_offsets_fit(m);
    if (st) st->round1_layout = (bp.bs.cmp ? 1 : 0) | (pk8 ? 2 : 0) | (xq ? 4 : 0) | (bp.bs.cmp == 2 ? 8 : 0);
    const uint64_t xqw = xq_words(1u << hb);
    uint32_t* xq_dh = nullptr;
    uint32_t* xq_pc = nullptr;
    uint32_t* xq_pn = nullptr;
    if (xq) {
        const uint64_t need = xqw + 1032 + 2ull * kXq * nb_tab;
        if (c->segx_words < need) {
            hipFree(c->segx);
            c->segx = nullptr;
            c->segx_words = 0;
            if (hipMalloc(&c->segx, need * 4) != hipSuccess) {
                (void)hipGetLastError();
                return set_err(SA_E_NOMEM, "second-pass queue workspace (%llu words)", (unsigned long long)need);
            }
            c->segx_words = need;
        }
        xq_dh = c->segx + xqw;
        xq_pc = xq_dh + 1032;
        xq_pn = xq_pc + (uint64_t)kXq * nb_tab;
    }
    uint32_t* const g_lo = os_ghist(c);
    uint32_t* const g_hi = os_ghist(c) + kLoRadix;
    const uint32_t stripes = padded ? text_stripes(c) : 1u;
    uint32_t* const cursor = stripes > 1 ? c->hist : os_ghist(c) + 5 * kRadix;
    uint32_t* const cursor_sum = stripes > 1 ? c->hist + kMaxStripes * kLoRadix : cursor;
    if (stripes > 1) SA_HIP(hipMemsetAsync(cursor, 0, (size_t)stripes * kLoRadix * 4, s));
    if (!padded) {
        tm.begin(SA_K_SCAN);
        hipLaunchKernelGGL(k_digit_base_wide, dim3(1), dim3(1024), 0, s, (const uint32_t*)g_lo, kLoRadix, os_base(c));
        tm.end();
    }
    tm.begin(SA_K_SCATTER_FIRST);
    {
        constexpr int kItemsA = SA_ITEMS_A;
        constexpr int kTextBlock = SA_TEXT_BLOCK;
        const bool pow2 = (bp.bs.sigma & (bp.bs.sigma - 1)) == 0;
        const bool dna = SA_DNA_SWAR && c->dna && bp.bs.s + bp.bs.R + kItemsA - 1 <= 32 && 2 * bp.bs.s <= 32;
        const bool ident = SA_TEXT_IDENT && bp.bs.sigma == 256 && bp.bs.s + bp.bs.R <= 8 && bp.bs.s <= 4;
        auto text_grid = [&](int block) {
            const uint64_t tile = (uint64_t)block * kItemsA;
            return (uint32_t)std::max<uint64_t>(
                1, std::min<uint64_t>((n + tile - 1) / tile, (uint64_t)c->cus * (kSpBlock / block)));
        };
#define SA_TEXT_PASS(P, PK, BLK, DNA, ID)                                                                     \
    hipLaunchKernelGGL((k_split_text<kItemsA, BLK, P, PK, DNA, ID>), dim3(text_grid(BLK)), dim3(BLK), 0, s, d_text, n, \
                       (const uint16_t*)c->code, bp.bs, (const uint32_t*)(padded ? pstart : os_base(c)),           \
                       os_tickets(c), c->keys[0], c->vals_alt, g_hi, cursor, m, blo, bhi,                          \
                       padded ? (const uint32_t*)pstart + 1 : nullptr, padded ? c->words + 11 : nullptr, hb, bp.ib, \
                       stripes)
        if (listed) {
            constexpr int kItemsL = SA_ITEMS_B, kListBlock = SA_LIST_BLOCK;
            const uint64_t tl = (uint64_t)kListBlock * kItemsL;
            const uint32_t gl = (uint32_t)std::max<uint64_t>(
                1, std::min<uint64_t>((m + tl - 1) / tl, (uint64_t)c->cus * (kSpBlock / kListBlock)));
            if (pk8)
                hipLaunchKernelGGL((k_split_list<kItemsL, kListBlock, true>), dim3(gl), dim3(kListBlock), 0, s, bp.bs,
                                   (const uint64_t*)lkeys, (const uint32_t*)lpos, m, blo, (const uint32_t*)os_base(c),
                                   os_tickets(c), c->keys[0], c->vals_alt, g_hi, cursor, hb, bp.ib,
                                   striped ? (const uint32_t*)rcur : nullptr, rcap);
            else
                hipLaunchKernelGGL((k_split_list<kItemsL, kListBlock, false>), dim3(gl), dim3(kListBlock), 0, s, bp.bs,
                                   (const uint64_t*)lkeys, (const uint32_t*)lpos, m, blo, (const uint32_t*)os_base(c),
                                   os_tickets(c), c->keys[0], c->vals_alt, g_hi, cursor, 0u, 0u,
                                   striped ? (const uint32_t*)rcur : nullptr, rcap);
        } else if (pk8 && np2) {
#define SA_TEXT_NP2(R32)                                                                                         \
    hipLaunchKernelGGL((k_split_text<kItemsA, kSpBlock, false, true, false, false, R32>), dim3(text_grid(kSpBlock)), \
                       dim3(kSpBlock), 0, s, d_text, n, (const uint16_t*)c->code, bp.bs,                           \
                       (const uint32_t*)(padded ? pstart : os_base(c)), os_tickets(c), c->keys[0], c->vals_alt, g_hi, \
                       cursor, m, blo, bhi, padded ? (const uint32_t*)pstart + 1 : nullptr,                        \
                       padded ? c->words + 11 : nullptr, hb, bp.ib, stripes)
            if (bp.bs.powR1 * (uint64_t)bp.bs.sigma <= 0xFFFFFFFFull && !(((uint32_t)c->tune >> 28) & 1u))
                SA_TEXT_NP2(true);
            else
                SA_TEXT_NP2(false);
#undef SA_TEXT_NP2
        } else if (pk8 && dna) {
            SA_TEXT_PASS(true, true, kTextBlock, true, false);
        } else if (pk8 && ident) {
            SA_TEXT_PASS(true, true, kTextBlock, false, true);
        } else if (pk8) {
            SA_TEXT_PASS(true, true, kTextBlock, false, false);
        } else if (pow2 && ident) {
            SA_TEXT_PASS(true, false, kTextBlock, false, true);
        } else if (pow2) {
            SA_TEXT_PASS(true, false, kTextBlock, false, false);
        } else if (bp.bs.powR1 * (uint64_t)bp.bs.sigma <= 0xFFFFFFFFull && !(((uint32_t)c->tune >> 28) & 1u)) {
            hipLaunchKernelGGL((k_split_text<kItemsA, kSpBlock, false, false, false, false, true>),
                               dim3(text_grid(kSpBlock)), dim3(kSpBlock), 0, s, d_text, n, (const uint16_t*)c->code,
                               bp.bs, (const uint32_t*)(padded ? pstart : os_base(c)), os_tickets(c), c->keys[0],
                               c->vals_alt, g_hi, cursor, m, blo, bhi, padded ? (const uint32_t*)pstart + 1 : nullptr,
                               padded ? c->words + 11 : nullptr, hb, bp.ib, stripes);
        } else {
            SA_TEXT_PASS(false, false, kSpBlock, false, false);
        }
#undef SA_TEXT_PASS
    }
    tm.end();
    add_bytes(st, SA_K_SCATTER_FIRST, listed ? (pk8 ? 20 : 24) * m : n + (pk8 ? 8 : 12) * m);
    tm.begin(SA_K_SCAN);
    hipLaunchKernelGGL(k_digit_base_wide, dim3(1), dim3(1024), 0, s, (const uint32_t*)g_hi, 1u << hb,
                       os_base(c) + kLoRadix);
    if (xq)
        hipLaunchKernelGGL(k_xq_dh, dim3(1), dim3(1024), 0, s, (const uint32_t*)g_hi, 1u << hb,
                           (c->dbg & SA_DEBUG_XQ_OVERFLOW) ? 1u : 0u, xq_dh);
    if (padded) {
        if (stripes > 1)
            hipLaunchKernelGGL(k_sum_rows, dim3(1), dim3(kLoRadix), 0, s, (const uint32_t*)cursor, stripes, cursor_sum);
        hipLaunchKernelGGL(k_digit_base_wide, dim3(1), dim3(1024), 0, s, (const uint32_t*)cursor_sum, kLoRadix, dlo);
    }
    tm.end();
    tm.begin(SA_K_SCATTER_KEYS);
    {
        constexpr int kItemsB = SA_ITEMS_B, kItemsPk = SA_ITEMS_PK;
        const SrcBucketKeys sb{c->keys[0], c->vals_alt, bp.bs.rb, bp.bs.bsh, bp.bs.cmul, blo};
        const SrcPk8 sp{c->keys[0]};
        uint32_t* tk = os_tickets(c) + 1;
        const uint32_t* hbase = os_base(c) + kLoRadix;
        SA_HIP(hipMemsetAsync(c->segw, 0, segw_words(1u << hb) * 4, s));
        SegXq sx;
        if (xq) {
            SA_HIP(hipMemsetAsync(c->segx, 0, xqw * 4, s));
            sx.cur = c->segx;
            sx.sbase = reinterpret_cast<uint64_t*>(c->segx + (uint64_t)kXq * kSegs * (1u << hb));
            sx.done = c->segx + 3ull * kXq * kSegs * (1u << hb);
            sx.tickets = sx.done + kXq * kSegs;
            sx.dh = xq_dh;
            sx.err2 = c->words + 9;
            sx.cap = (uint32_t)std::min<uint64_t>(c->kucap, UINT32_MAX);
        }
        constexpr int kSegBlock = SA_SEG_BLOCK;
        const int sblk = hb <= 9 ? kSegBlock : kSpBlock;
        const uint64_t ut = (uint64_t)sblk * (pk8 ? kItemsPk : kItemsB);
        const uint64_t units = (m + ut - 1) / ut + kSegs;
        const uint32_t grid = xq ? (uint32_t)c->cus * (kSpBlock / sblk)
                                 : (uint32_t)std::max<uint64_t>(1, std::min<uint64_t>(units, (uint64_t)c->cus * (kSpBlock / sblk)));
        switch (hb) {
#define SA_SEG_LAUNCH(S, B, SRC, SH, IT)                                                                      \
    if (xq)                                                                                                   \
        hipLaunchKernelGGL((k_split_seg<S, B, IT, (B <= 9 ? kSegBlock : kSpBlock), true>), dim3(grid),        \
                           dim3(B <= 9 ? kSegBlock : kSpBlock), 0, s, SRC, m, SH,                              \
                           (const uint32_t*)(padded ? pstart : os_base(c)), hbase, c->segw, tk, bp.ib, c->keys_u,      \
                           c->words + 4, padded ? (const uint32_t*)cursor : nullptr,                           \
                           padded ? (const uint32_t*)dlo : nullptr, stripes, sx);                              \
    else                                                                                                      \
        hipLaunchKernelGGL((k_split_seg<S, B, IT, (B <= 9 ? kSegBlock : kSpBlock)>), dim3(grid),                \
                           dim3(B <= 9 ? kSegBlock : kSpBlock), 0, s, SRC, m, SH,                              \
                           (const uint32_t*)(padded ? pstart : os_base(c)), hbase, c->segw, tk, bp.ib, c->keys_u,      \
                           c->words + 4, padded ? (const uint32_t*)cursor : nullptr,                           \
                           padded ? (const uint32_t*)dlo : nullptr, stripes)
#define SA_SEG_PASS(B)                                                                                        \
    case B:                                                                                                   \
        if (pk8) SA_SEG_LAUNCH(SrcPk8, B, sp, 64u - B, kItemsPk);                                             \
        else SA_SEG_LAUNCH(SrcBucketKeys, B, sb, kLoBits, kItemsB);                                           \
        break;
            SA_SEG_PASS(7)
            SA_SEG_PASS(8)
            SA_SEG_PASS(9)
            SA_SEG_PASS(10)
#undef SA_SEG_PASS
#undef SA_SEG_LAUNCH
            default: return set_err(SA_E_INTERNAL, "second bucket pass of %u bits", hb);
        }
        const uint32_t gb = (uint32_t)std::min<uint64_t>(((uint64_t)nb_tab + kBlock) / kBlock, 1024);
        uint32_t* bstart = c->segw + kBstartOff;
        uint32_t* bdmin = bstart + kBstartWords;
#define SA_BSTARTS(R)                                                                                         \
    if (xq)                                                                                                   \
        hipLaunchKernelGGL(k_bucket_starts_xq<R>, dim3(R), dim3(kLoRadix), 0, s, hbase, (const uint32_t*)sx.cur, \
                           (const uint32_t*)xq_dh, m, bp.bs.cmul, bp.bs.bsh, bstart, bdmin, xq_pc, xq_pn, blo); \
    else                                                                                                      \
        hipLaunchKernelGGL(k_bucket_starts<R>, dim3(gb), dim3(kBlock), 0, s, (const uint32_t*)(padded ? dlo : os_base(c)), \
                           hbase, (const uint32_t*)c->segw, m, bp.bs.cmul, bp.bs.bsh, bstart, bdmin, blo)
        switch (hb) {
            case 7: SA_BSTARTS(128); break;
            case 8: SA_BSTARTS(256); break;
            case 9: SA_BSTARTS(512); break;
            default: SA_BSTARTS(1024); break;
        }
#undef SA_BSTARTS
    }
    tm.end();
    add_bytes(st, SA_K_SCATTER_KEYS, (pk8 ? 16 : 20) * m);
    SA_HIP(hipGetLastError());
    const uint64_t nw = (m + kWinStride - 1) / kWinStride;
    uint32_t* ws = c->vals_alt;
    uint32_t* list = c->vals_alt + nw + 1;
    tm.begin(SA_K_WINDOWS);
    {
        const uint32_t g1 = (uint32_t)std::min<uint64_t>((nw + kBlock) / kBlock, 8192);
        hipLaunchKernelGGL(k_window_starts_tab, dim3(g1), dim3(kBlock), 0, s, (const uint32_t*)(c->segw + kBstartOff),
                           nb_tab, m, nw, ws, list + 4 * nw + 2);
        const uint32_t g2 = (uint32_t)std::min<uint64_t>((nw + kBlock - 1) / kBlock, 1024);
        hipLaunchKernelGGL(k_window_list, dim3(g2), dim3(kBlock), 0, s, (const uint32_t*)ws, nw, list, c->words);
    }
    tm.end();
    add_bytes(st, SA_K_WINDOWS, 8 * nw);
    SA_HIP(hipGetLastError());
    SA_HIP(hipMemcpyAsync(c->host_words, c->words, 48, hipMemcpyDeviceToHost, s));
    uint32_t* skew = list + nw;
    uint32_t* cnt_u = skew + nw;
    uint32_t* cnt_g = cnt_u + nw + 1;
    uint32_t* const rank_arr = br_.rank ? br_.rank : c->rank;
    uint32_t* const member = br_.member ? br_.member : c->member;
    SA_HIP(hipEventRecord(c->ev[kSyncEv], s));
    SA_HIP(hipMemsetAsync(cnt_u, 0, (2 * nw + 2) * 4, s));
    SA_HIP(hipMemsetAsync(member, 0, (n + 31) / 32 * 4, s));
    SA_HIP(host_sync_event(c->ev[kSyncEv]));
    if (c->host_words[4]) return set_err(SA_E_INTERNAL, "radix look-back did not complete");
    if (padded && c->host_words[11]) {
        SA_TRACE("  bucketed round 1: padded segment overflow, again with exact digit totals");
        const int rc = round1_bucketed(c, d_text, n, d_sa, bp, br_, s, tm, st, done, fused, seg, ksh, false, allow_xq,
                                       round2);
        if (st) st->round1_segments = 2;
        return rc;
    }
    if (xq && c->host_words[9]) {
        SA_TRACE("  bucketed round 1: second-pass queue overflow, again with one region");
        return round1_bucketed(c, d_text, n, d_sa, bp, br_, s, tm, st, done, fused, seg, ksh, allow_pad, false,
                               round2);
    }
    if (st) st->largest_window = (int32_t)std::min<uint32_t>(c->host_words[5], INT32_MAX);
    if (c->host_words[5] > (uint32_t)kBsCap) {
        SA_TRACE("  bucketed round 1: window of %u > %d suffixes, full sort instead", c->host_words[5], kBsCap);
        return SA_OK;
    }
    BucketRel br{cnt_g + nw + 1, c->segw + kBstartOff, c->segw + kBstartOff + kBstartWords, bp.bs.rb};
    br.bits1 = bits1;
    SegOut so{rank_arr, member, br_.sa_off, c->u_pos[1], c->u_idx[1], c->u_g[1], cnt_u, cnt_g, kKeySample};
    so.tmp_rank = br_.prefix ? br_.tmp_rank : nullptr;
    so.samples = (SA_LAZY_SAMPLES && !br_.always_u && !(c->dbg & SA_DEBUG_NO_KEY1_ROUND)) ? 0u : 1u;
    uint32_t* const retry = cnt_g + 2 * nw + 2;
    BucketRel br_measured = br;
    br_measured.bits1 = 0;
    uint4* const hdr = reinterpret_cast<uint4*>(((uintptr_t)(retry + nw + 4) + 15) & ~(uintptr_t)15);
    uint32_t* const hx = xq ? reinterpret_cast<uint32_t*>(hdr + nw + 1) : nullptr;
    constexpr uint32_t kBsRows = (kBsBlock / kWave) * kBsItems;
    uint32_t* const xrows = xq ? hx + 16 * (nw + 1) : nullptr;
    const uint64_t* const wide_in = xq ? c->keys[1] : c->keys_u;
    auto local_sort = [&](const SegOut& o) {
        const uint32_t g = std::max<uint32_t>(1, std::min(c->host_words[7], kBsGrid));
        static_assert(kRetryWord == kUsFlagWord + 1, "one memset clears words[12..15]");
        (void)hipMemsetAsync(c->words + kUsFlagWord, 0, 16, s);
        if (fast32) {
            const uint32_t gs = (uint32_t)std::max<uint64_t>(1, std::min<uint64_t>((nw + kBlock - 1) / kBlock, 1024));
            const bool cr = xq && !(((uint32_t)c->tune >> 29) & 1u);
            const uint32_t ls_grid = (c->dbg & SA_DEBUG_LS_ONE_WG) ? 1u : kBsWpc * (uint32_t)c->cus;
            hipLaunchKernelGGL(k_window_split, dim3(gs), dim3(kBlock), 0, s, (const uint32_t*)list, (const uint32_t*)ws,
                               br, c->words, hdr, retry, 1u, (const uint32_t*)xq_pc, (const uint32_t*)xq_pn, nb_tab, hx,
                               cr ? kBsRows : 0u);
            if (xq) {
                if (cr)
                    hipLaunchKernelGGL(k_window_rows<true>, dim3(2048), dim3(kBlock), 0, s, (const uint32_t*)c->words,
                                       (const uint4*)hdr, (const uint32_t*)hx, kBsRows, xrows);
                else
                    hipLaunchKernelGGL(k_window_rows<false>, dim3(2048), dim3(kBlock), 0, s, (const uint32_t*)c->words,
                                       (const uint4*)hdr, (const uint32_t*)hx, kBsRows, xrows);
                XqWin xw;
                xw.hx = hx;
                xw.rows = xrows;
#define SA_LS_XQ(V, CR)                                                                                          \
    hipLaunchKernelGGL((k_bucket_sort<kBsBlock, kBsItems, NoProbe, true, V, CR>), dim3(ls_grid), dim3(kBsBlock), 0, \
                       s, (const uint64_t*)c->keys_u, (const uint4*)hdr, bp.bs.rb, br.bits1, bp.ib, c->words,      \
                       c->keys[0], d_sa, retry, o, xw)
                switch (ls_variant(c) | (cr ? 4 : 0)) {
                case 1: SA_LS_XQ(1, false); break;
                case 2: SA_LS_XQ(2, false); break;
                case 3: SA_LS_XQ(3, false); break;
                case 4: SA_LS_XQ(0, true); break;
                case 5: SA_LS_XQ(1, true); break;
                case 6: SA_LS_XQ(2, true); break;
                case 7: SA_LS_XQ(3, true); break;
                default: SA_LS_XQ(0, false); break;
                }
#undef SA_LS_XQ
                hipLaunchKernelGGL(k_window_gather, dim3(1024), dim3(kBlock), 0, s, (const uint32_t*)retry,
                                   (const uint32_t*)c->words, (const uint32_t*)ws, (const uint32_t*)br.wb,
                                   (const uint32_t*)xq_pc, (const uint32_t*)xq_pn, nb_tab, (const uint64_t*)c->keys_u,
                                   c->keys[1]);
            } else {
#define SA_LS(V)                                                                                                 \
    hipLaunchKernelGGL((k_bucket_sort<kBsBlock, kBsItems, NoProbe, false, V>), dim3(ls_grid), dim3(kBsBlock), 0, \
                       s, (const uint64_t*)c->keys_u, (const uint4*)hdr, bp.bs.rb, br.bits1, bp.ib, c->words,   \
                       c->keys[0], d_sa, retry, o)
                switch (ls_variant(c)) {
                case 1: SA_LS(1); break;
                case 2: SA_LS(2); break;
                case 3: SA_LS(3); break;
                default: SA_LS(0); break;
                }
#undef SA_LS
// ... 116 lines not shown
```

hpc_suffix_array_amd/csrc/sa_split.h:

```cpp
#pragma once
#include <type_traits>
#include "sa_bucket.h"
#include "sa_onesweep.h"

#ifndef SA_SEG_PROF
#define SA_SEG_PROF 0
#endif
#ifndef SA_TEXT_PROF
#define SA_TEXT_PROF 0
#endif

namespace sa {

constexpr int kSpBlock = 1024;
constexpr int kSpItems = 8;
constexpr int kSpTile = kSpBlock * kSpItems;
constexpr int kSpWaves = kSpBlock / kWave;

__device__ __forceinline__ uint32_t wave_min_u32(uint32_t x) {
#pragma unroll
    for (int o = kWave / 2; o > 0; o >>= 1) x = min(x, (uint32_t)__shfl_xor((int)x, o, kWave));
    return x;
}
__device__ __forceinline__ uint32_t wave_max_u32(uint32_t x) {
// ... 169 lines not shown
        load(tn < tiles ? tn : tiles - 1, kn, vn);
        stamp(2);
#pragma unroll
        for (int j = 0; j < ITEMS; ++j) {
            const uint32_t d = dr[j] >> 16;
            if (d < (uint32_t)RADIX) {
                const uint32_t pos = s_start[d] + (dr[j] & 0x3FFFu);
                s_keys[pos] = k[j];
                s_vals[pos] = v[j];
            }
        }
        __syncthreads();
        if (dg < (uint32_t)RADIX) s_cnt[dg] = 0;
        if (STABLE && dg < 3u) s_nx[dg] = ~0u;
        stamp(3);
#pragma unroll
        for (int j = 0; j < ITEMS; ++j) {
            const uint32_t q = j * kSpBlock + dg;
            if (q < valid) {
                const uint64_t key = s_keys[q];
                const uint32_t dd = src_digit(src, key, shift, mask, 0);
                const uint64_t g = (uint64_t)s_gofs[dd] + (q - s_start[dd]);
                if (g < n) {
                    out_keys[g] = key;
                    out_vals[g] = s_vals[q];
                }
            }
        }
        __syncthreads();
        stamp(4);
#pragma unroll
        for (int j = 0; j < ITEMS; ++j) {
            k[j] = kn[j];
            v[j] = vn[j];
        }
        t = tn;
        par ^= 1u;
    }
    if constexpr (PROF) {
        if (dg == 0)
            for (int q = 0; q < 5; ++q) atomicAdd(reinterpret_cast<unsigned long long*>(err + 2) + q, tacc[q]);
        if (dg < (uint32_t)RADIX) {
            atomicAdd(reinterpret_cast<unsigned long long*>(err + 12), (unsigned long long)lbsteps[0]);
            atomicAdd(reinterpret_cast<unsigned long long*>(err + 14), (unsigned long long)lbsteps[1]);
        }
    }
}

#ifndef SA_DNA_SWAR
#define SA_DNA_SWAR 1
#endif
#ifndef SA_TEXT_IDENT
#define SA_TEXT_IDENT 1
#endif
#ifndef SA_TEXT_FULL
#define SA_TEXT_FULL 1
#endif
#ifndef SA_TEXT_LOAD16
#define SA_TEXT_LOAD16 1
#endif
#ifndef SA_TEXT_SCAN1
#define SA_TEXT_SCAN1 1
#endif
#ifndef SA_TEXT_TAB1
#define SA_TEXT_TAB1 1
#endif
#ifndef SA_TEXT_EARLY
#define SA_TEXT_EARLY 1
#endif
#ifndef SA_TEXT_TPT
#define SA_TEXT_TPT 4
#endif
template <int ITEMS, int BLOCK = kSpBlock, bool POW2 = false, bool PK8 = false, bool DNA = false, bool IDENT = false,
          bool R32 = false>
__global__ __launch_bounds__(BLOCK, 2048 / BLOCK) void k_split_text(const uint8_t* __restrict__ text, uint64_t n,
                                                         const uint16_t* __restrict__ code, BucketSpec b,
                                                         const uint32_t* __restrict__ digit_base,
                                                         uint32_t* __restrict__ ticket, uint64_t* __restrict__ out_keys,
                                                         uint32_t* __restrict__ out_vals,
                                                         uint32_t* __restrict__ ghist_hi, uint32_t* __restrict__ cursor,
                                                         uint64_t m, uint32_t blo, uint32_t bhi,
                                                         const uint32_t* __restrict__ seg_end = nullptr,
                                                         uint32_t* __restrict__ ovf = nullptr, uint32_t pk_hb = 0,
                                                         uint32_t pk_ib = 0, uint32_t stripes = 1) {
    constexpr bool NP2 = PK8 && !POW2;
    constexpr int RADIX = kLoRadix;
    constexpr int RWAVES = RADIX / kWave;
    constexpr int TILE = BLOCK * ITEMS;
    constexpr int kHalo = kMaxK;
    constexpr int NW = (TILE + kHalo) / 4;
    constexpr int WPT = (NW + BLOCK - 1) / BLOCK;
    static_assert(ITEMS % 4 == 0 && kHalo % 4 == 0 && TILE <= 65535, "word staging, 16-bit tile offsets");
    constexpr bool LD16 = SA_TEXT_LOAD16 != 0, SCAN1 = SA_TEXT_SCAN1 != 0, TAB1 = SA_TEXT_TAB1 != 0;
    constexpr bool EARLY = SA_TEXT_EARLY != 0;
    constexpr int NC = NW / 4;
    static_assert(!LD16 || (NW % 4 == 0 && NC <= BLOCK && WPT <= 4), "one 16-byte chunk per lane");
    static_assert(!SCAN1 || RADIX == 4 * kWave, "wave 0 scans four digits per lane");
    __shared__ uint64_t s_keys[TILE];
    __shared__ uint16_t s_idx[TILE];
    __shared__ __attribute__((aligned(16))) uint32_t s_dcw[(DNA && LD16) ? 4 : NW + 8];
    __shared__ uint32_t s_pkw[DNA ? (NW + 3) / 4 + 4 : 1];
    __shared__ uint8_t s_map[256];
    __shared__ __attribute__((aligned(16))) uint32_t s_cnt[RADIX];
    __shared__ __attribute__((aligned(8))) uint16_t s_start[RADIX];
    constexpr uint32_t kTabSkip = ~0u;
    __shared__ uint32_t s_gofs[RADIX];
    __shared__ uint32_t s_tmp[RWAVES];
    __shared__ uint32_t s_tile[2];
    __shared__ uint32_t s_kept;
    __shared__ uint32_t s_hhi[1024];
    __shared__ uint32_t s_gend[RADIX];
    const uint8_t* s_dc = reinterpret_cast<const uint8_t*>(s_dcw);
    const uint32_t bspan = bhi - blo;
    bool over = false;

    const uint32_t wave = wave_id(), lane = lane_id();
    const uint32_t dg = threadIdx.x;
    const uint64_t tiles = (n + TILE - 1) / TILE;
    const uint32_t K = b.s + b.R;
    const uint32_t stripe = blockIdx.x % stripes;
    uint32_t sbase = 0;
    for (uint32_t i = dg; i < 1024u; i += BLOCK) s_hhi[i] = 0;
    if (seg_end && dg < (uint32_t)RADIX) {
        const uint32_t lo = digit_base[dg], hi = seg_end[dg], sc = (hi - lo) / stripes;
        sbase = lo + stripe * sc;
        s_gend[dg] = stripe + 1 == stripes ? hi : sbase + sc;
    }
    cursor += stripe * RADIX;
    if (dg < 256u) {
        const uint32_t cv = code[dg];
        s_map[dg] = (uint8_t)(cv ? cv - 1u : 0u);
    }
    if (dg < (uint32_t)RADIX) s_cnt[dg] = 0;
    constexpr uint32_t TPT = SA_TEXT_TPT;
    static_assert(TPT >= 1 && (TPT & (TPT - 1)) == 0, "tiles per ticket: a power of two");
    const uint32_t tpt = tiles >= 128ull * gridDim.x ? TPT : tiles >= 32ull * gridDim.x && TPT > 1 ? TPT / 2 : 1u;
    uint32_t tk_tile = 0, tk_left = 0;
    auto next_tile = [&]() -> uint32_t {
        if constexpr (TPT == 1) {
            return atomicAdd(ticket, 1u);
        } else {
            if (tk_left == 0) {
                tk_tile = atomicAdd(ticket, 1u) * tpt;
                tk_left = tpt;
            }
            --tk_left;
            return tk_tile++;
        }
    };
    if (dg == 0) {
        s_tile[0] = next_tile();
        if constexpr (EARLY) s_tile[1] = next_tile();
    }
    __syncthreads();
    uint64_t t = (uint32_t)__builtin_amdgcn_readfirstlane((int)s_tile[0]);
    auto load4 = [&](uint64_t pos) -> uint32_t {
        if (pos + 4 <= n && (((uintptr_t)(text + pos)) & 3) == 0) return *reinterpret_cast<const uint32_t*>(text + pos);
        uint32_t w = 0;
        for (int q = 0; q < 4; ++q)
            if (pos + q < n) w |= (uint32_t)text[pos + q] << (8 * q);
        return w;
    };
    const uint32_t t_whole = n >= 4ull * NW ? (uint32_t)((n - 4ull * NW) / TILE + 1) : 0u;
    uint32_t raw[LD16 ? 4 : WPT];
    const bool al16 = (((uintptr_t)text) & 15) == 0;
    auto load = [&](uint64_t tt) {
        const uint64_t tb = tt * TILE;
        if constexpr (LD16) {
            const uint64_t cb = tb + 16ull * (dg < (uint32_t)NC ? dg : (uint32_t)NC - 1u);
            if (al16 && (uint32_t)tt < t_whole) {
                const uint4 v = *reinterpret_cast<const uint4*>(text + cb);
                raw[0] = v.x, raw[1] = v.y, raw[2] = v.z, raw[3] = v.w;
            } else {
#pragma unroll
                for (int i = 0; i < 4; ++i) raw[i] = load4(cb + 4ull * i);
            }
        } else {
#pragma unroll
            for (int i = 0; i < WPT; ++i) {
                const uint32_t w = dg + i * BLOCK;
                raw[i] = load4(tb + 4ull * (w < (uint32_t)NW ? w : (uint32_t)NW - 1u));
            }
        }
    };
    if (t < tiles) load(t);
    uint32_t par = 0;
    const uint32_t t_int = n >= (uint64_t)TILE + K ? (uint32_t)((n - TILE - K) / TILE + 1) : 0u;
    const uint32_t t_last = (uint32_t)(tiles - 1);
#if SA_TEXT_PROF
    uint64_t pacc[5] = {0, 0, 0, 0, 0}, plast = clock64();
#define TEXT_STAMP(k)                               \
    if (dg == 0) {                                  \
        const uint64_t now_ = clock64();            \
        pacc[k] += now_ - plast;                    \
        plast = now_;                               \
    }
#else
#define TEXT_STAMP(k)
#endif
    auto stage = [&](uint64_t tt) {
        const uint64_t tb = tt * TILE;
        const bool whole = (uint32_t)tt < t_whole;
        if constexpr (LD16) {
            if (dg < (uint32_t)NC) {
                uint32_t o[4];
#pragma unroll
                for (int i = 0; i < 4; ++i) {
                    o[i] = 0;
                    if (whole) {
                        if constexpr (DNA)
                            o[i] = ((raw[i] >> 1) ^ (raw[i] >> 2)) & 0x03030303u;
                        else if constexpr (IDENT)
                            o[i] = raw[i];
                        else
                            o[i] = (uint32_t)s_map[raw[i] & 0xFFu] | ((uint32_t)s_map[(raw[i] >> 8) & 0xFFu] << 8) |
                                   ((uint32_t)s_map[(raw[i] >> 16) & 0xFFu] << 16) |
                                   ((uint32_t)s_map[raw[i] >> 24] << 24);
                    } else {
#pragma unroll
                        for (int q = 0; q < 4; ++q) {
                            const uint64_t pos = tb + 16ull * dg + 4ull * i + q;
                            o[i] |= (pos < n ? (uint32_t)s_map[(raw[i] >> (8 * q)) & 0xFFu] : 0u) << (8 * q);
                        }
                    }
                }
                if constexpr (DNA) {
                    uint32_t pw = 0;
#pragma unroll
                    for (int i = 0; i < 4; ++i)
                        pw |= ((((o[i] & 3u) << 6) | ((o[i] >> 4) & 0x30u) | ((o[i] >> 14) & 0xCu) | (o[i] >> 24)) & 0xFFu)
                              << (8 * i);
                    s_pkw[dg] = pw;
                } else {
                    *reinterpret_cast<uint4*>(&s_dcw[4 * dg]) = make_uint4(o[0], o[1], o[2], o[3]);
                }
            }
        } else {
#pragma unroll
        for (int i = 0; i < WPT; ++i) {
            const uint32_t w = dg + i * BLOCK;
            if (w < (uint32_t)NW) {
                uint32_t o = 0;
                if (whole) {
                    if constexpr (DNA)
                        o = ((raw[i] >> 1) ^ (raw[i] >> 2)) & 0x03030303u;
                    else if constexpr (IDENT)
                        o = raw[i];
                    else
                        o = (uint32_t)s_map[raw[i] & 0xFFu] | ((uint32_t)s_map[(raw[i] >> 8) & 0xFFu] << 8) |
                            ((uint32_t)s_map[(raw[i] >> 16) & 0xFFu] << 16) | ((uint32_t)s_map[raw[i] >> 24] << 24);
                } else {
#pragma unroll
                    for (int q = 0; q < 4; ++q) {
                        const uint64_t pos = tb + 4ull * w + q;
                        o |= (pos < n ? (uint32_t)s_map[(raw[i] >> (8 * q)) & 0xFFu] : 0u) << (8 * q);
                    }
                }
                s_dcw[w] = o;
                if constexpr (DNA)
                    reinterpret_cast<uint8_t*>(s_pkw)[w] =
                        (uint8_t)(((o & 3u) << 6) | ((o >> 4) & 0x30u) | ((o >> 14) & 0xCu) | (o >> 24));
            }
        }
        }
    };
    if constexpr (EARLY) {
        if (t < tiles) stage(t);
        __syncthreads();
    }
    while (t < tiles) {
        const uint64_t tb = t * TILE;
        const uint32_t valid = (uint32_t)t < t_last ? (uint32_t)TILE : (uint32_t)(n - tb);
        if constexpr (!EARLY) {
            stage(t);
            if (dg == 0) s_tile[par ^ 1u] = next_tile();
            __syncthreads();
        }
        TEXT_STAMP(0)
        const bool full0 = SA_TEXT_FULL && valid == (uint32_t)TILE && blo == 0 && bspan == (1u << b.bb);
        uint64_t k[ITEMS];
        uint32_t dr[ITEMS];
        {
            const uint32_t l0 = ITEMS * dg;
            uint32_t D = 0;
            using RT = typename std::conditional<R32 && !POW2, uint32_t, uint64_t>::type;
            RT r = 0;
            const uint32_t lg = POW2 ? (uint32_t)__builtin_ctz(b.sigma) : 0u;
            const uint32_t dmask = POW2 ? (lg * b.s >= 32 ? ~0u : (1u << (lg * b.s)) - 1u) : 0u;
            const uint64_t rmask = POW2 ? ((1ull << (lg * b.R)) - 1ull) : 0ull;
            const uint32_t bksh = POW2 ? lg * b.s - b.bb : 0u;
            const uint64_t mulR = b.cmp == 2 ? 1u : b.cmp ? 2u : b.R + 1u, addR = b.cmp == 2 ? 0u : b.cmp ? 1u : b.s + b.R;
            uint64_t win = 0;
            uint32_t wid[IDENT ? ITEMS / 4 + 2 : 1];
            if constexpr (IDENT) {
#pragma unroll
                for (int q = 0; q < ITEMS / 4 + 2; ++q) wid[q] = s_dcw[l0 / 4 + q];
            } else if constexpr (DNA) {
                const uint32_t bo = l0 / 4, sh = bo & 3u;
                const uint32_t w0 = s_pkw[bo >> 2], w1 = s_pkw[(bo >> 2) + 1], w2 = s_pkw[(bo >> 2) + 2];
                win = ((uint64_t)__builtin_bswap32(__builtin_amdgcn_alignbyte(w1, w0, sh)) << 32) |
                      __builtin_bswap32(__builtin_amdgcn_alignbyte(w2, w1, sh));
            } else if constexpr (POW2) {
                for (uint32_t q = 0; q < b.s; ++q) D = (D << lg) | s_dc[l0 + q];
                for (uint32_t q = 0; q < b.R; ++q) r = (r << lg) | s_dc[l0 + b.s + q];
            } else {
                for (uint32_t q = 0; q < b.s; ++q) D = D * b.sigma + s_dc[l0 + q];
                for (uint32_t q = 0; q < b.R; ++q) r = r * (RT)b.sigma + s_dc[l0 + b.s + q];
            }
            const bool interior = (uint32_t)t < t_int;
            const bool full = full0 && interior;
            uint32_t xo[ITEMS / 4], xm[ITEMS / 4], xn[ITEMS / 4];
            if constexpr (!DNA && !IDENT) {
                lds_bytes<ITEMS>(s_dcw, l0, xo);
                lds_bytes<ITEMS>(s_dcw, l0 + b.s, xm);
                lds_bytes<ITEMS>(s_dcw, l0 + K, xn);
            }
            const uint32_t dsh = 64u - 2u * b.s, rsh = 64u - 2u * K;
            auto keyloop = [&](auto fullc) {
            constexpr bool FULL = decltype(fullc)::value;
#pragma unroll
            for (int j = 0; j < ITEMS; ++j) {
                if constexpr (DNA) {
                    const uint64_t x = win << (2 * j);
                    D = (uint32_t)(x >> dsh);
                    r = (x >> rsh) & rmask;
                } else if constexpr (IDENT) {
                    const uint64_t x =
                        ((uint64_t)__builtin_bswap32(__builtin_amdgcn_alignbyte(wid[j / 4 + 1], wid[j / 4], j % 4)) << 32) |
                        __builtin_bswap32(__builtin_amdgcn_alignbyte(wid[j / 4 + 2], wid[j / 4 + 1], j % 4));
                    D = (uint32_t)(x >> (64u - 8u * b.s));
                    r = (x >> (64u - 8u * K)) & rmask;
                } else if (j > 0) {
                    const uint32_t xi = byte_at<ITEMS>(xm, j - 1);
                    if constexpr (POW2) {
                        D = ((D << lg) | xi) & dmask;
                        r = ((r << lg) | byte_at<ITEMS>(xn, j - 1)) & rmask;
                    } else {
                        D = (D - byte_at<ITEMS>(xo, j - 1) * (uint32_t)b.pow_s1) * b.sigma + xi;
                        r = (r - (RT)xi * (RT)b.powR1) * (RT)b.sigma + byte_at<ITEMS>(xn, j - 1);
                    }
                }
                const uint64_t low = (FULL || interior) ? (uint64_t)r * mulR + addR : bucket_low(b, r, n - (tb + l0 + j));
                k[j] = ((uint64_t)D << b.rb) | low;
                const uint32_t bk = POW2 ? (D >> bksh) : (uint32_t)(((uint64_t)D * (uint32_t)b.cmul) >> b.bsh);
                const uint32_t lb = bk - blo;
                if constexpr (FULL) {
// ... 271 lines not shown
        __syncthreads();
        const uint64_t tn = (uint32_t)__builtin_amdgcn_readfirstlane((int)s_tile[par ^ 1u]);
        uint64_t kn[ITEMS];
        uint32_t vn[ITEMS];
        uint64_t tbn;
        uint32_t validn;
        locate(tn < tiles ? tn : tiles - 1, tbn, validn);
        load(tbn, validn, kn, vn);
        const uint32_t kbsh = b.rb + (PK8 ? (uint32_t)__builtin_ctz(b.sigma) * b.s - b.bb : 0u);
        const uint64_t remmask = PK8 ? (1ull << kbsh) - 1ull : 0ull;
#pragma unroll
        for (int j = 0; j < ITEMS; ++j) {
            const uint32_t d = dr[j] >> 16;
            if (d < (uint32_t)RADIX) {
                const uint32_t q = s_start[d] + (dr[j] & 0xFFFFu);
                if constexpr (PK8) {
                    const uint32_t hi = ((uint32_t)(k[j] >> kbsh) - blo) >> kLoBits;
                    s_keys[q] = ((uint64_t)hi << (64u - pk_hb)) | ((k[j] & remmask) << pk_ib) | v[j];
                    s_pos[q] = d;
                } else {
                    s_keys[q] = k[j];
                    s_pos[q] = v[j];
                }
            }
        }
        __syncthreads();
#pragma unroll
        for (int j = 0; j < ITEMS; ++j) {
            const uint32_t q = j * BLOCK + dg;
            if (q < valid) {
                const uint64_t key = s_keys[q];
                const uint32_t dd =
                    PK8 ? s_pos[q] : (bucket_of(key, b.rb, b.cmul, b.bsh) - blo) & (RADIX - 1);
                const uint64_t g = (uint64_t)s_gofs[dd] + (q - s_start[dd]);
                if (g < m) {
                    out_keys[g] = key;
                    if constexpr (!PK8) out_vals[g] = s_pos[q];
                }
            }
        }
        __syncthreads();
#pragma unroll
        for (int j = 0; j < ITEMS; ++j) {
            k[j] = kn[j];
            v[j] = vn[j];
        }
        t = tn;
        tb = tbn;
        valid = validn;
        par ^= 1u;
    }
    for (uint32_t i = dg; i < 1024u; i += BLOCK)
        if (s_hhi[i]) atomicAdd(&ghist_hi[i], s_hhi[i]);
}

constexpr uint32_t kSegs = kLoRadix;
constexpr uint32_t kMaxStripes = 8;
constexpr uint64_t segw_words(int radix) { return 3ull * kSegs * radix + kSegs; }
constexpr uint64_t kBstartOff = segw_words(1024);
constexpr uint64_t kBstartWords = (1ull << 18) + 1;

constexpr uint32_t kXqSlack = 2048;
constexpr uint32_t kXqTicketStride = 32;
struct SegXq {
    uint32_t* cur = nullptr;
    uint64_t* sbase = nullptr;
    uint32_t* done = nullptr;
    uint32_t* tickets = nullptr;
    const uint32_t* dh = nullptr;
    uint32_t cap = 0;
    uint32_t* err2 = nullptr;
};
constexpr uint64_t xq_words(int radix) { return 3ull * kXq * kSegs * radix + kXq * kSegs + kXq * kXqTicketStride; }

template <class Src, int RBITS, int ITEMS, int BLOCK = kSpBlock, bool XQ = false>
__global__ __launch_bounds__(BLOCK, 2048 / BLOCK) void k_split_seg(Src src, uint64_t n, uint32_t shift,
                                                        const uint32_t* __restrict__ lo_base,
                                                        const uint32_t* __restrict__ digit_base,
                                                        uint32_t* __restrict__ segw, uint32_t* __restrict__ ticket,
                                                        uint32_t ib, uint64_t* __restrict__ out_w,
                                                        uint32_t* __restrict__ err,
                                                        const uint32_t* __restrict__ seg_cnt = nullptr,
                                                        const uint32_t* __restrict__ dense_lo = nullptr,
                                                        uint32_t stripes = 1, SegXq xq = SegXq{}) {
    constexpr int RADIX = 1 << RBITS;
    constexpr int RWAVES = RADIX / kWave;
    constexpr int WTILE = kWave * ITEMS;
    constexpr int TILE = BLOCK * ITEMS;
    static_assert(BLOCK >= RADIX && (int)kSegs <= BLOCK, "one thread per digit / segment");
    static_assert((int)(kSegs * kMaxStripes) <= 2 * BLOCK, "two sub-segments per thread in the unit numbering");
    static_assert(TILE <= 65535, "16-bit tile offsets");
    __shared__ uint64_t s_keys[TILE];
    __shared__ uint16_t s_dig[TILE];
    __shared__ uint32_t s_dmin[RADIX];
    __shared__ uint32_t s_cnt[RADIX];
    __shared__ uint16_t s_start[RADIX];
    __shared__ uint32_t s_gofs[RADIX];
    __shared__ uint32_t s_tmp[(BLOCK / kWave)];
    __shared__ uint32_t s_ubase[kSegs * kMaxStripes + 1];
    __shared__ uint32_t s_tile[2];
    __shared__ uint32_t s_last;
    __shared__ uint32_t s_claim[RADIX];
    const uint32_t xqq = XQ ? (blockIdx.x & (kXq - 1)) : 0u;
    uint32_t* const cur = XQ ? xq.cur + (uint64_t)xqq * kSegs * RADIX : segw;
    uint64_t* const sbase = XQ ? xq.sbase + (uint64_t)xqq * kSegs * RADIX
                               : reinterpret_cast<uint64_t*>(segw + (uint64_t)kSegs * RADIX);
    uint32_t* const done = XQ ? xq.done + xqq * kSegs : segw + 3ull * kSegs * RADIX;
    if constexpr (XQ) ticket = xq.tickets + xqq * kXqTicketStride;
    const uint64_t gcap = XQ ? (uint64_t)xq.cap : n;
    const uint32_t xrs = XQ ? xq.dh[RADIX] : 0u;
    constexpr uint64_t kReady = 1ull << 32;

    const uint32_t wave = wave_id(), lane = lane_id();
    const uint32_t dg = threadIdx.x;
    const uint32_t mask = RADIX - 1;
    const uint32_t nsub = kSegs * stripes;
    auto sub_lo = [&](uint32_t q) -> uint64_t {
        const uint32_t l = q / stripes, sidx = q % stripes;
        if (stripes == 1) return lo_base[l];
        return (uint64_t)lo_base[l] + sidx * ((lo_base[l + 1] - lo_base[l]) / stripes);
    };
    auto sub_hi = [&](uint32_t q) -> uint64_t {
        const uint32_t l = q / stripes, sidx = q % stripes;
        if (seg_cnt) return sub_lo(q) + seg_cnt[sidx * kSegs + l];
        return l + 1 < kSegs ? (uint64_t)lo_base[l + 1] : n;
    };
    const uint32_t* const dlo = dense_lo ? dense_lo : lo_base;
    {
        uint32_t x0 = 0, x1 = 0;
        const uint32_t q0 = 2 * dg, q1 = 2 * dg + 1;
        if (q0 < nsub) x0 = (uint32_t)((sub_hi(q0) - sub_lo(q0) + TILE - 1) / TILE);
        if (q1 < nsub) x1 = (uint32_t)((sub_hi(q1) - sub_lo(q1) + TILE - 1) / TILE);
        const uint32_t x = x0 + x1;
        const uint32_t inc = wave_inclusive_sum(x);
        if (lane == kWave - 1) s_tmp[wave] = inc;
        __syncthreads();
        uint32_t off = 0;
        for (uint32_t w = 0; w < wave; ++w) off += s_tmp[w];
        if (q0 < nsub) s_ubase[q0] = off + inc - x;
        if (q1 < nsub) s_ubase[q1] = off + inc - x1;
        if (q1 + 1 >= nsub && q0 < nsub) s_ubase[nsub] = off + inc;
    }
    if (dg < (uint32_t)RADIX) s_cnt[dg] = 0;
    if (dg == 0) s_tile[0] = atomicAdd(ticket, 1u);
    __syncthreads();
    const uint32_t units = s_ubase[nsub];
    auto qcount = [&](uint32_t U) -> uint32_t { return XQ ? (U + (kXq - 1) - xqq) / kXq : U; };
    auto unit_of = [&](uint32_t t) -> uint32_t { return XQ ? t * kXq + xqq : t; };
    auto units_of = [&](uint32_t l) -> uint32_t {
        return qcount(s_ubase[(l + 1) * stripes]) - qcount(s_ubase[l * stripes]);
    };
    auto locate = [&](uint32_t u, uint32_t& l, uint64_t& tb, uint32_t& valid) {
        uint32_t a = 0, b = nsub;
        while (b - a > 1) {
            const uint32_t mid = (a + b) / 2;
            if (s_ubase[mid] <= u) a = mid;
            else b = mid;
        }
        l = a / stripes;
        tb = sub_lo(a) + (uint64_t)(u - s_ubase[a]) * TILE;
        const uint64_t e = sub_hi(a);
        valid = (uint32_t)(e - tb < (uint64_t)TILE ? e - tb : (uint64_t)TILE);
    };
    uint64_t k[ITEMS];
    uint32_t v[ITEMS];
    auto load = [&](uint64_t tb, uint32_t valid, uint64_t* kk, uint32_t* vv) {
        const uint32_t last = valid - 1;
// ... 223 lines not shown
```

include/sa_hip.h:

```cpp
#ifndef SA_HIP_H
#define SA_HIP_H

#include <stdint.h>

#ifdef __cplusplus
extern "C" {
#endif

#define SA_OK 0
#define SA_E_INVALID (-1)
#define SA_E_NOMEM (-2)
#define SA_E_HIP (-3)
#define SA_E_INTERNAL (-4)

#define SA_MAX_ROUNDS 64

enum sa_kernel_kind {
    SA_K_INIT = 0,
    SA_K_HIST_FIRST = 1,
    SA_K_HIST_KEYS = 2,
    SA_K_SCAN = 3,
    SA_K_SCATTER_FIRST = 4,
    SA_K_SCATTER_KEYS = 5,
    SA_K_HEADS = 6,
    SA_K_HEADS_SCAN = 7,
    SA_K_RERANK = 8,
    SA_K_SEG_COUNT = 9,
    SA_K_SEG_SCAN = 10,
    SA_K_SEG_WRITE = 11,
    SA_K_ALPHABET = 12,
    SA_K_PACK = 13,
    SA_K_SORT_U = 14,
    SA_K_WINDOWS = 15,
    SA_K_LOCAL_SORT = 16,
    SA_K_PIVOT_KEYS = 17,
    SA_K_PIVOT_COUNT = 18,
    SA_K_PIVOT_WRITE = 19,
    SA_K_COUNT = 20
};

#define SA_ROUND1_AUTO 0
#define SA_ROUND1_LSD 1
#define SA_ROUND1_BUCKETED 2
#define SA_ROUND1_PIVOT 3

#define SA_SCHEDULE_PACKED 0
#define SA_SCHEDULE_REFERENCE 1

#define SA_DEBUG_NO_CMP 0x1u
#define SA_DEBUG_NO_PK8 0x2u
#define SA_DEBUG_NO_PAD 0x4u
#define SA_DEBUG_PAD_OVERFLOW 0x8u
#define SA_DEBUG_NO_FAST32 0x10u
#define SA_DEBUG_NO_PIVOT 0x20u
#define SA_DEBUG_PERM_ALWAYS 0x40u
#define SA_DEBUG_NO_XQ 0x80u
#define SA_DEBUG_XQ_OVERFLOW 0x100u
#define SA_DEBUG_NO_KEY1_ROUND 0x400u
#define SA_DEBUG_NO_TIED 0x200u
#define SA_DEBUG_NO_EONLY 0x800u
#define SA_DEBUG_EONLY 0x1000u
#define SA_DEBUG_FAST32_SMALL 0x2000u
#define SA_DEBUG_NO_ROUND2_FUSED 0x4000u
#define SA_DEBUG_LS_ONE_WG 0x8000u

typedef struct {
    int32_t profile;
    int32_t schedule;
    int32_t init_chars;
    int32_t radix;
    int32_t round1;
    uint32_t debug;
    int32_t span_extra;
    int32_t tune;
} sa_opts;

typedef struct {
    int32_t rounds;
    int32_t n_kinds;
    double total_ms;
    double h2d_ms, d2h_ms;
    double round_ms[SA_MAX_ROUNDS];
    uint64_t distinct[SA_MAX_ROUNDS];
    int32_t passes[SA_MAX_ROUNDS];
    uint64_t sorted_n[SA_MAX_ROUNDS];
    uint64_t prefix_len[SA_MAX_ROUNDS];
    int32_t schedule;
    int32_t init_chars;
    int32_t sigma;
    int32_t sparse_ranks;
    int32_t round1;
    int32_t largest_window;
    uint64_t model_bytes;
    double kern_ms[SA_K_COUNT];
    uint64_t kern_launches[SA_K_COUNT];
    uint64_t kern_bytes[SA_K_COUNT];
    int32_t round1_segments;
    int32_t round1_layout;
    uint64_t round_bytes[SA_MAX_ROUNDS];
    int32_t round1_windows[4];
} sa_stats;

typedef struct sa_context sa_context;

int sa_context_create(int device, uint64_t max_n, sa_context** out);
int sa_context_set_debug(sa_context* ctx, const sa_opts* opts);
void sa_context_destroy(sa_context* ctx);
uint64_t sa_workspace_bytes(uint64_t max_n);

int sa_build_device(sa_context* ctx, const uint8_t* d_text, uint64_t n, uint32_t* d_sa,
                    void* stream, const sa_opts* opts, sa_stats* stats);

int sa_build_ex(const uint8_t* text, uint64_t n, void* sa_out, int sa_width,
                const sa_opts* opts, sa_stats* stats);

int sa_check_device(sa_context* ctx, const uint8_t* d_text, uint64_t n, const uint32_t* d_sa,
                    void* stream);
int sa_check(const uint8_t* text, uint64_t n, const void* sa, int sa_width);

int sa_lcp_device(sa_context* ctx, const uint8_t* d_text, uint64_t n, const uint32_t* d_sa, uint32_t* d_lcp,
                  uint64_t* lrs_len, uint64_t* lrs_pos, void* stream);
int sa_lcp(const uint8_t* text, uint64_t n, const void* sa, int sa_width, void* lcp_out, uint64_t* lrs_len,
           uint64_t* lrs_pos);


#define SA_FIND_LANE 1u
#define SA_FIND_WAVE 2u
#define SA_FIND_LANE_MAX 3584

int sa_find_device(const uint8_t* d_text, uint64_t n, const uint32_t* d_sa,
                   const uint8_t* d_pat, uint64_t pat_bytes, const uint64_t* d_pat_off ,
                   uint64_t nq, uint32_t* d_lo, uint32_t* d_hi, uint32_t flags, void* stream);
int sa_find(const uint8_t* text, uint64_t n, const void* sa, int sa_width,
            const uint8_t* pat, const uint64_t* pat_off, uint64_t nq,
            uint64_t* lo_out, uint64_t* hi_out);
int sa_find_ex(const uint8_t* text, uint64_t n, const void* sa, int sa_width,
               const uint8_t* pat, const uint64_t* pat_off, uint64_t nq,
               uint64_t* lo_out, uint64_t* hi_out, uint32_t flags);

int sa_match_device(const uint8_t* d_text, uint64_t n, const uint32_t* d_sa,
                    const uint8_t* d_pat, uint64_t pat_bytes, const uint64_t* d_pat_off ,
                    uint64_t nq, uint32_t* d_len, uint32_t* d_lo, uint32_t* d_hi, uint32_t flags, void* stream);
int sa_matching_stats_device(const uint8_t* d_text, uint64_t n, const uint32_t* d_sa,
                             const uint8_t* d_query, uint64_t m, uint64_t max_len ,
                             uint32_t* d_len, uint32_t* d_lo, uint32_t* d_hi ,
                             uint32_t flags, void* stream);
int sa_match(const uint8_t* text, uint64_t n, const void* sa, int sa_width,
             const uint8_t* pat, const uint64_t* pat_off, uint64_t nq,
             uint64_t* len_out, uint64_t* lo_out, uint64_t* hi_out, uint32_t flags);
int sa_matching_stats(const uint8_t* text, uint64_t n, const void* sa, int sa_width,
                      const uint8_t* query, uint64_t m, uint64_t max_len,
                      uint64_t* len_out, uint64_t* lo_out, uint64_t* hi_out, uint32_t flags);

#define SA_BWT_STATS 258

int sa_bwt_device(const uint8_t* d_text, uint64_t n, const uint32_t* d_sa, uint8_t* d_bwt,
                  uint64_t* d_stats , void* stream);
int sa_bwt(const uint8_t* text, uint64_t n, const void* sa, int sa_width, uint8_t* bwt_out,
           uint64_t* stats_out );

int sa_inverse_device(sa_context* ctx, uint64_t n, const uint32_t* d_sa, uint32_t* d_isa, void* stream);
int sa_inverse(const void* sa, uint64_t n, int sa_width, void* isa_out );

#define SA_LOCATE_SA_ORDER 1u
#define SA_LOCATE_SMALL_CHUNKS 2u
#define SA_LOCATE_TILE 2048

int sa_locate_device(sa_context* ctx, uint64_t n, const uint32_t* d_sa, const uint32_t* d_lo, const uint32_t* d_hi,
                     uint64_t nq, uint64_t max_hits, uint32_t flags, uint64_t* d_off ,
                     uint32_t* d_pos , uint64_t pos_cap, uint64_t* total, void* stream);
int sa_locate(const void* sa, uint64_t n, int sa_width, const uint64_t* lo, const uint64_t* hi, uint64_t nq,
              uint64_t max_hits, uint32_t flags, uint64_t* off_out , void* pos_out, uint64_t pos_cap);


int sa_alphabet_device(const uint8_t* d_text, uint64_t n, uint32_t present_out[8], void* stream);

int sa_pack_keys_device(sa_context* ctx, const uint8_t* d_text, uint64_t n, uint64_t lo, uint64_t hi,
                        const uint16_t code[256], uint64_t base, uint32_t K, uint64_t* d_keys_out,
                        void* stream);

int sa_sort_pairs_device(sa_context* ctx, const uint64_t* d_keys_in, const uint32_t* d_vals_in, uint64_t m,
                         uint32_t bits, uint64_t* d_keys_out, uint32_t* d_vals_out, void* stream);

int sa_scatter_u64_device(uint64_t* d_dst, uint64_t dst_n, const int64_t* d_idx, int64_t base,
                          const uint64_t* d_src, uint64_t m, void* stream);

int sa_gather_u64_device(uint64_t* d_dst, const uint64_t* d_src, uint64_t src_n, const int64_t* d_idx, int64_t base,
                         uint64_t m, void* stream);

int sa_running_max_i64_device(int64_t* d_v, uint64_t m, void* stream);
int sa_inclusive_sum_i64_device(int64_t* d_v, uint64_t m, void* stream);
int sa_count_below_u64_device(const uint64_t* d_sorted, uint64_t m, const uint64_t* d_q, uint64_t nq, int right,
                              int64_t* d_out, void* stream);
int sa_select_u8_device(const uint8_t* d_mask, uint64_t m, int64_t* d_out, uint64_t* count, void* stream);

#define SA_DIST_OK 0
#define SA_DIST_UNSUPPORTED 1
#define SA_DIST_UNBALANCED 2

typedef struct {
    int32_t status;
    int32_t sigma;
    int32_t K;
    int32_t bucket_bits;
    uint64_t m;
    uint64_t sa_off;
    uint64_t m_max;
    uint32_t bucket_lo, bucket_hi;
    int32_t round1_ok;
    int32_t reserved;
    uint64_t heads;
    uint64_t unsorted;
    uint64_t groups;
} sa_dist_info;

int sa_dist_begin(sa_context* ctx, const uint8_t* d_text, uint64_t n, int world, int rank,
                  const uint32_t present[8], uint64_t* d_coarse, void* stream, sa_dist_info* info);
int sa_dist_cuts(sa_context* ctx, const uint64_t* h_coarse, sa_dist_info* info);
int sa_dist_reserve(sa_context* ctx, uint64_t max_n, int world);
int sa_dist_release(sa_context* ctx);
int sa_dist_plan_cuts(int world, uint64_t n, int bucket_bits, const uint64_t* h_coarse, uint32_t* cuts_out,
                      uint64_t* m_max);
int sa_dist_round1(sa_context* ctx, uint32_t* d_sa_local, void* stream, sa_dist_info* info, sa_stats* stats);
int sa_dist_req_count(sa_context* ctx, uint64_t h, uint64_t* counts_out, void* stream, sa_dist_info* info);
int sa_dist_req_fill(sa_context* ctx, uint64_t h, uint32_t* d_req, void* stream);
int sa_dist_answer(sa_context* ctx, const uint32_t* d_req, uint64_t nreq, uint64_t* d_ans, void* stream);
int sa_dist_refine(sa_context* ctx, uint64_t h, const uint64_t* d_ans, uint32_t* d_sa_local, void* stream,
                   sa_dist_info* info);

int sa_generate_text_device(uint8_t* d_out, uint64_t n, uint64_t seed, const uint8_t* alphabet,
                            uint32_t sigma, void* stream);

const char* sa_last_error(void);
int sa_device_count(void);
const char* sa_version(void);
uint64_t sa_host_syncs(void);

uint64_t sa_struct_size(int which);

#ifdef __cplusplus
}
#endif

#endif
```

Measured before the change: 109.7 billion.

## Sample the alphabet scan and verify speculatively inside bucketed round 1

For large inputs the alphabet kernel now reads only a sample of the text: the head, the tail, and the first 4 KiB of every 64 KiB block, rather than every byte. The bucketed round-1 stage kernel checks each mapped byte against the sampled code table and raises a miss flag plus a stop ticket if it finds a byte outside it. When that happens, round 1 reruns with the exact full-text alphabet scan. This removes most of the full-text alphabet read, at the cost of extra per-byte checking in the stage kernel and a full redo when the sample misses a symbol.

```diff
diff --git a/hpc_suffix_array_amd/_native.py b/hpc_suffix_array_amd/_native.py
--- a/hpc_suffix_array_amd/_native.py
+++ b/hpc_suffix_array_amd/_native.py
@@ -44,7 +44,8 @@
                "sa_locate_device", "sa_locate",
                "sa_dist_begin", "sa_dist_cuts", "sa_dist_plan_cuts", "sa_dist_reserve", "sa_dist_release", "sa_dist_round1", "sa_dist_req_count", "sa_dist_req_fill",
                "sa_dist_answer", "sa_dist_refine",
-               "sa_last_error", "sa_host_syncs", "sa_device_count", "sa_version", "sa_struct_size"]
+               "sa_last_error", "sa_host_syncs", "sa_device_count", "sa_version", "sa_struct_size",
+               "sa_alphabet_sampled"]
 
 
 class SAError(RuntimeError):
@@ -55,7 +56,7 @@
                "no_pivot": 0x20, "perm_always": 0x40, "no_xq": 0x80, "xq_overflow": 0x100,
                "no_tied": 0x200, "no_key1_round": 0x400, "no_eonly": 0x800,
                "eonly": 0x1000, "fast32_small": 0x2000, "no_round2_fused": 0x4000,
-               "ls_one_wg": 0x8000}
+               "ls_one_wg": 0x8000, "alpha_sample": 0x10000, "alpha_exact": 0x20000}
 
 
 def debug_bits(names) -> int:
@@ -99,6 +100,7 @@
         ("round1_layout", ctypes.c_int32),
         ("round_bytes", ctypes.c_uint64 * SA_MAX_ROUNDS),
         ("round1_windows", ctypes.c_int32 * 4),
+        ("alphabet_mode", ctypes.c_int32),
     ]
 
     def to_dict(self) -> dict:
@@ -126,6 +128,7 @@
             "reference_model_bytes": int(self.model_bytes),
             "round_bytes": [int(x) for x in self.round_bytes[:r]],
             "round1_windows": [int(x) for x in self.round1_windows],
+            "alphabet_mode": self.alphabet_mode,
             "kernels": {k: {"ms": self.kern_ms[i], "launches": int(self.kern_launches[i]),
                             "bytes": int(self.kern_bytes[i])} for i, k in enumerate(KERNEL_KINDS)},
         }
@@ -265,6 +268,8 @@
     L.sa_last_error.restype = ctypes.c_char_p
     L.sa_host_syncs.argtypes = []
     L.sa_host_syncs.restype = ctypes.c_uint64
+    L.sa_alphabet_sampled.argtypes = [u64, u64]
+    L.sa_alphabet_sampled.restype = i32
     L.sa_device_count.argtypes = []
     L.sa_device_count.restype = i32
     L.sa_version.argtypes = []
diff --git a/hpc_suffix_array_amd/csrc/sa_build.hip b/hpc_suffix_array_amd/csrc/sa_build.hip
--- a/hpc_suffix_array_amd/csrc/sa_build.hip
+++ b/hpc_suffix_array_amd/csrc/sa_build.hip
@@ -158,6 +158,8 @@
     int32_t tune = 0;
     bool dna = false;
     bool samples_pending = false;
+    bool alpha_prove = false;
+    bool alpha_refuted = false;
 };
 
 namespace sa {
@@ -798,7 +800,7 @@
     tm.begin(SA_K_ALPHABET);
     {
         const uint32_t grid = (uint32_t)std::min<uint64_t>((n + kBlock * 16 - 1) / (kBlock * 16), SA_ALPHA_GRID);
-        hipLaunchKernelGGL(k_alphabet, dim3(grid), dim3(kBlock), 0, s, d_text, n, c->alpha);
+        hipLaunchKernelGGL(k_alphabet, dim3(grid), dim3(kBlock), 0, s, d_text, n, c->alpha, 0u);
     }
     tm.end();
     add_bytes(st, SA_K_ALPHABET, n);
@@ -1255,64 +1257,91 @@
     tm.round_mark();
     uint32_t* h_alpha = c->host_words + 64;
     uint16_t* h_code = reinterpret_cast<uint16_t*>(c->host_words + 320);
-    SA_HIP(hipMemsetAsync(c->alpha, 0, 8 * 4, s));
-    tm.begin(SA_K_ALPHABET);
-    {
-        const uint32_t grid = (uint32_t)std::min<uint64_t>((n + kBlock * 16 - 1) / (kBlock * 16), SA_ALPHA_GRID);
-        hipLaunchKernelGGL(k_alphabet, dim3(grid), dim3(kBlock), 0, s, d_text, n, c->alpha);
-    }
-    tm.end();
-    SA_HIP(hipGetLastError());
-    add_bytes(st, SA_K_ALPHABET, n);
-    SA_HIP(hipMemcpyAsync(h_alpha, c->alpha, 8 * 4, hipMemcpyDeviceToHost, s));
     const uint32_t tail_n = (uint32_t)std::min<uint64_t>(n, (uint64_t)kMaxK);
     uint8_t* h_tail = reinterpret_cast<uint8_t*>(c->host_words + 2048);
-    SA_HIP(hipMemcpyAsync(h_tail, d_text + (n - tail_n), tail_n, hipMemcpyDeviceToHost, s));
-    SA_HIP(host_sync(s));
-    uint32_t sigma = 0;
-    for (int b = 0; b < 256; ++b) h_code[b] = ((h_alpha[b >> 5] >> (b & 31)) & 1u) ? (uint16_t)(++sigma) : 0;
-    SA_HIP(hipMemcpyAsync(c->code, h_code, 256 * 2, hipMemcpyHostToDevice, s));
-    c->dna = sigma == 4 && h_code['A'] && h_code['C'] && h_code['G'] && h_code['T'];
-    uint32_t K = choose_chars(sigma, n, opts ? opts->init_chars : 0);
-    const uint64_t base = (uint64_t)sigma + 1;
+    bool sampled = !(c->dbg & SA_DEBUG_ALPHA_EXACT) && !c->alpha_refuted &&
+                   (n >= kAlphaMinN || (c->dbg & SA_DEBUG_ALPHA_SAMPLE));
+    int alpha_mode = sampled ? 1 : 0;
+    bool allow_bucketed = true;
+    uint32_t sigma = 0, K = 0, Kb = 0;
+    uint64_t base = 0;
     const Chunking ch = plan_chunks(n);
     uint64_t* keys1 = nullptr;
     uint32_t ksh1 = 0;
-    c->samples_pending = false;
     uint32_t P = 0;
-
     BucketPlan bp;
     const int r1 = opts ? opts->round1 : SA_ROUND1_AUTO;
-    const uint32_t Kb = (opts && opts->init_chars > 0) || sigma <= 1 ? K : min_chars(sigma, n);
-    bool bucketed = plan_bucketed(sigma, n, Kb, r1, c->radix, &bp, 1, (c->dbg & SA_DEBUG_NO_CMP) ? 0 : 1);
-    if (bucketed && bp.bs.cmp && short_suffix_ties(h_tail, n, tail_n, h_code, sigma, bp.bs.s, bp.bs.R))
-        bucketed = plan_bucketed(sigma, n, Kb, r1, c->radix, &bp, 1, 0);
-    const bool force_eonly = (c->dbg & SA_DEBUG_EONLY) != 0;
-    if (bucketed && bp.bs.cmp == 1 && ((sigma & (sigma - 1)) != 0 || force_eonly) && !(c->dbg & SA_DEBUG_NO_EONLY)) {
-        const uint32_t hb = bp.bs.bb - kLoBits;
-        BucketPlan b2;
-        if ((force_eonly || !plan_pk8(bp, hb, c->dbg, true)) && plan_bucketed(sigma, n, Kb, r1, c->radix, &b2, 1, 2) &&
-            (force_eonly || plan_pk8(b2, hb, c->dbg, true)) &&
-            !short_suffix_ties(h_tail, n, tail_n, h_code, sigma, b2.bs.s, b2.bs.R, b2.K))
-            bp = b2;
-    }
+    bool bucketed = false;
     bool fused = false;
     bool r1_pivot = false;
     uint64_t D = 0, m = 0, G = 0;
     uint64_t seg1[3] = {0, 0, 0};
     int r2 = 0;
-    if (bucketed) {
-        bool done = false;
-        rc = round1_bucketed(c, d_text, n, d_sa, bp, full_range(bp, n), s, tm, st, &done, &fused, seg1, &ksh1, true,
-                             true, &r2);
-        if (rc) return rc;
-        bucketed = done;
-        if (done) {
-            keys1 = c->keys[0];
-            P = 2;
-            K = bp.K;
-        }
-    }
+    for (;;) {
+        SA_HIP(hipMemsetAsync(c->alpha, 0, 8 * 4, s));
+        tm.begin(SA_K_ALPHABET);
+        {
+            const uint64_t chunks = sampled ? alpha_chunks(n) : (n + 15) / 16;
+            const uint32_t grid = (uint32_t)std::min<uint64_t>((chunks + kBlock - 1) / kBlock, SA_ALPHA_GRID);
+            hipLaunchKernelGGL(k_alphabet, dim3(grid), dim3(kBlock), 0, s, d_text, n, c->alpha, sampled ? 1u : 0u);
+        }
+        tm.end();
+        SA_HIP(hipGetLastError());
+        add_bytes(st, SA_K_ALPHABET, sampled ? alpha_sample_bytes(n) : n);
+        SA_HIP(hipMemcpyAsync(h_alpha, c->alpha, 8 * 4, hipMemcpyDeviceToHost, s));
+        SA_HIP(hipMemcpyAsync(h_tail, d_text + (n - tail_n), tail_n, hipMemcpyDeviceToHost, s));
+        SA_HIP(host_sync(s));
+        sigma = 0;
+        for (int b = 0; b < 256; ++b) h_code[b] = ((h_alpha[b >> 5] >> (b & 31)) & 1u) ? (uint16_t)(++sigma) : 0;
+        SA_HIP(hipMemcpyAsync(c->code, h_code, 256 * 2, hipMemcpyHostToDevice, s));
+        c->dna = sigma == 4 && h_code['A'] && h_code['C'] && h_code['G'] && h_code['T'];
+        K = choose_chars(sigma, n, opts ? opts->init_chars : 0);
+        base = (uint64_t)sigma + 1;
+        c->samples_pending = false;
+
+        Kb = (opts && opts->init_chars > 0) || sigma <= 1 ? K : min_chars(sigma, n);
+        bucketed = allow_bucketed &&
+                   plan_bucketed(sigma, n, Kb, r1, c->radix, &bp, 1, (c->dbg & SA_DEBUG_NO_CMP) ? 0 : 1);
+        if (bucketed && bp.bs.cmp && short_suffix_ties(h_tail, n, tail_n, h_code, sigma, bp.bs.s, bp.bs.R))
+            bucketed = plan_bucketed(sigma, n, Kb, r1, c->radix, &bp, 1, 0);
+        const bool force_eonly = (c->dbg & SA_DEBUG_EONLY) != 0;
+        if (bucketed && bp.bs.cmp == 1 && ((sigma & (sigma - 1)) != 0 || force_eonly) &&
+            !(c->dbg & SA_DEBUG_NO_EONLY)) {
+            const uint32_t hb = bp.bs.bb - kLoBits;
+            BucketPlan b2;
+            if ((force_eonly || !plan_pk8(bp, hb, c->dbg, true)) &&
+                plan_bucketed(sigma, n, Kb, r1, c->radix, &b2, 1, 2) && (force_eonly || plan_pk8(b2, hb, c->dbg, true)) &&
+                !short_suffix_ties(h_tail, n, tail_n, h_code, sigma, b2.bs.s, b2.bs.R, b2.K))
+                bp = b2;
+        }
+        if (sampled && !bucketed) {
+            sampled = false;
+            alpha_mode = 0;
+            continue;
+        }
+        if (bucketed) {
+            bool done = false;
+            c->alpha_prove = sampled;
+            rc = round1_bucketed(c, d_text, n, d_sa, bp, full_range(bp, n), s, tm, st, &done, &fused, seg1, &ksh1, true,
+                                 true, &r2);
+            c->alpha_prove = false;
+            if (rc) return rc;
+            if (sampled && !done) {
+                sampled = false;
+                alpha_mode = c->alpha_refuted ? 2 : 0;
+                allow_bucketed = c->alpha_refuted;
+                continue;
+            }
+            bucketed = done;
+            if (done) {
+                keys1 = c->keys[0];
+                P = 2;
+                K = bp.K;
+            }
+        }
+        break;
+    }
+    if (st) st->alphabet_mode = alpha_mode;
     if (!bucketed) {
         const uint32_t bits1 = key_bits(base, K);
         SA_TRACE("packed: sigma=%u K=%u bits=%u", sigma, K, bits1);
@@ -2410,7 +2439,7 @@
     SA_HIP(hipMallocAsync((void**)&d_mask, 32, s));
     SA_HIP(hipMemsetAsync(d_mask, 0, 32, s));
     const uint32_t grid = (uint32_t)std::min<uint64_t>((n + kBlock * 16 - 1) / (kBlock * 16), 2048);
-    hipLaunchKernelGGL(k_alphabet, dim3(grid), dim3(kBlock), 0, s, d_text, n, d_mask);
+    hipLaunchKernelGGL(k_alphabet, dim3(grid), dim3(kBlock), 0, s, d_text, n, d_mask, 0u);
     SA_HIP(hipGetLastError());
     SA_HIP(hipMemcpyAsync(present_out, d_mask, 32, hipMemcpyDeviceToHost, s));
     SA_HIP(hipFreeAsync(d_mask, s));
diff --git a/hpc_suffix_array_amd/csrc/sa_dropin.cpp b/hpc_suffix_array_amd/csrc/sa_dropin.cpp
--- a/hpc_suffix_array_amd/csrc/sa_dropin.cpp
+++ b/hpc_suffix_array_amd/csrc/sa_dropin.cpp
@@ -7,6 +7,7 @@
 
 #include "../../include/sa_hip.h"
 #include "../../include/suffix_array.h"
+#include "sa_limits.h"
 
 static_assert(sizeof(SuffixArray) == 32, "SuffixArray must keep the reference's 32-byte layout");
 static_assert(offsetof(SuffixArray, n) == 8 && offsetof(SuffixArray, sa) == 16 && offsetof(SuffixArray, lcp) == 24,
@@ -88,6 +89,8 @@
 
 }
 
+extern "C" int sa_alphabet_sampled(uint64_t pos, uint64_t n) { return sa::alpha_sampled(pos, n) ? 1 : 0; }
+
 extern "C" uint64_t sa_struct_size(int which) {
     return which == 0 ? sizeof(sa_stats) : which == 1 ? sizeof(sa_opts) : 0;
 }
diff --git a/hpc_suffix_array_amd/csrc/sa_kernels.h b/hpc_suffix_array_amd/csrc/sa_kernels.h
--- a/hpc_suffix_array_amd/csrc/sa_kernels.h
+++ b/hpc_suffix_array_amd/csrc/sa_kernels.h
@@ -2,6 +2,7 @@
 #include <hip/hip_runtime.h>
 #include <stdint.h>
 
+#include "sa_limits.h"
 #include "sa_search.h"
 
 namespace sa {
@@ -662,19 +663,23 @@
 
 
 __global__ __launch_bounds__(kBlock) void k_alphabet(const uint8_t* __restrict__ text, uint64_t n,
-                                                     uint32_t* __restrict__ present) {
+                                                     uint32_t* __restrict__ present, uint32_t sampled) {
     __shared__ uint32_t s_m[kBlock * 9];
     uint32_t* m = s_m + threadIdx.x * 9;
 #pragma unroll
     for (int i = 0; i < 8; ++i) m[i] = 0;
     auto add = [&](uint32_t b) { atomicOr(&m[b >> 5], 1u << (b & 31u)); };
-    const uint64_t stride = (uint64_t)gridDim.x * kBlock * 16;
-    auto whole = [&](uint64_t i) { return i + 16 <= n && (((uintptr_t)(text + i)) & 15) == 0; };
-    uint64_t i = ((uint64_t)blockIdx.x * kBlock + threadIdx.x) * 16;
+    static_assert(kAlphaChunk == 16, "one uint4 per chunk");
+    const uint64_t vstride = (uint64_t)gridDim.x * kBlock;
+    const uint64_t nv = sampled ? alpha_chunks(n) : (n + 15) / 16;
+    auto at = [&](uint64_t c) { return sampled ? alpha_chunk_pos(c, n) : c * 16; };
+    auto whole = [&](uint64_t i) { return i < n && i + 16 <= n && (((uintptr_t)(text + i)) & 15) == 0; };
+    uint64_t cv = (uint64_t)blockIdx.x * kBlock + threadIdx.x;
+    uint64_t i = cv < nv ? at(cv) : kAlphaSkip;
     uint4 v = make_uint4(0u, 0u, 0u, 0u);
-    if (i < n && whole(i)) v = *reinterpret_cast<const uint4*>(text + i);
+    if (whole(i)) v = *reinterpret_cast<const uint4*>(text + i);
     uint32_t step = 0;
-    for (; i < n; i += stride) {
+    for (; cv < nv; cv += vstride) {
         if (step && (step & (step - 1)) == 0) {
             uint32_t all = ~0u;
 #pragma unroll
@@ -687,9 +692,9 @@
             if (all == ~0u) break;
         }
         ++step;
-        const uint64_t in = i + stride;
+        const uint64_t in = cv + vstride < nv ? at(cv + vstride) : kAlphaSkip;
         uint4 vn = make_uint4(0u, 0u, 0u, 0u);
-        if (in < n && whole(in)) vn = *reinterpret_cast<const uint4*>(text + in);
+        if (whole(in)) vn = *reinterpret_cast<const uint4*>(text + in);
         if (whole(i)) {
             const uint32_t w4[4] = {v.x, v.y, v.z, v.w};
             uint32_t o = v.x | v.y | v.z | v.w, a = v.x & v.y & v.z & v.w;
@@ -710,10 +715,11 @@
 #pragma unroll
                     for (int b = 0; b < 4; ++b) add((w4[q] >> (8 * b)) & 0xFFu);
             }
-        } else {
+        } else if (i != kAlphaSkip) {
             for (uint64_t j = i; j < n && j < i + 16; ++j) add(text[j]);
         }
         v = vn;
+        i = in;
     }
     __shared__ uint32_t s_or[8];
     if (threadIdx.x < 8) s_or[threadIdx.x] = 0;
@@ -749,6 +755,7 @@
 
 constexpr int kPackRun = kTile / kBlock;
 constexpr int kMaxK = 64;
+static_assert((uint64_t)kMaxK + kAlphaChunk <= kAlphaEdge, "the alphabet sample's tail holds the text's last kMaxK bytes");
 constexpr int kPackMaxPasses = 8;
 
 __global__ __launch_bounds__(kBlock) void k_pack_text(const uint8_t* __restrict__ text, uint64_t avail,
diff --git a/hpc_suffix_array_amd/csrc/sa_limits.h b/hpc_suffix_array_amd/csrc/sa_limits.h
--- a/hpc_suffix_array_amd/csrc/sa_limits.h
+++ b/hpc_suffix_array_amd/csrc/sa_limits.h
@@ -13,4 +13,62 @@
 
 constexpr bool xq_offsets_fit(uint64_t m) { return xq_region_space(m) <= 0xFFFFFFFFull; }
 
+constexpr uint64_t kAlphaEdge = 1ull << 16;
+constexpr uint64_t kAlphaBlock = 1ull << 16;
+constexpr uint64_t kAlphaHead = 1ull << 12;
+constexpr uint64_t kAlphaChunk = 16;
+constexpr uint64_t kAlphaMinN = 1ull << 24;
+constexpr uint64_t kAlphaSkip = ~0ull;
+static_assert(kAlphaEdge == kAlphaBlock && kAlphaHead % kAlphaChunk == 0 && kAlphaEdge % kAlphaChunk == 0,
+              "block 0 is the head; ranges are whole chunks");
+
+constexpr bool alpha_whole(uint64_t n) { return n <= 2 * kAlphaEdge; }
+constexpr uint64_t alpha_tail_start(uint64_t n) {
+    return alpha_whole(n) ? n : (n - kAlphaEdge) & ~(kAlphaChunk - 1);
 }
+constexpr uint64_t alpha_blocks(uint64_t n) { return alpha_whole(n) ? 0 : (alpha_tail_start(n) - 1) / kAlphaBlock; }
+
+constexpr bool alpha_sampled(uint64_t pos, uint64_t n) {
+    if (pos >= n) return false;
+    return alpha_whole(n) || pos < kAlphaEdge || pos >= alpha_tail_start(n) || (pos & (kAlphaBlock - 1)) < kAlphaHead;
+}
+
+constexpr uint64_t alpha_range_count(uint64_t n) { return n == 0 ? 0 : alpha_whole(n) ? 1 : alpha_blocks(n) + 2; }
+constexpr void alpha_range(uint64_t n, uint64_t r, uint64_t* lo, uint64_t* hi) {
+    const uint64_t T = alpha_tail_start(n), nb = alpha_blocks(n);
+    if (alpha_whole(n)) {
+        *lo = 0, *hi = n;
+    } else if (r == 0) {
+        *lo = 0, *hi = kAlphaEdge;
+    } else if (r <= nb) {
+        *lo = r * kAlphaBlock;
+        *hi = *lo + kAlphaHead < T ? *lo + kAlphaHead : T;
+    } else {
+        *lo = T, *hi = n;
+    }
+}
+constexpr uint64_t alpha_sample_bytes(uint64_t n) {
+    if (alpha_whole(n)) return n;
+    const uint64_t T = alpha_tail_start(n), nb = alpha_blocks(n);
+    const uint64_t last = nb ? (nb * kAlphaBlock + kAlphaHead < T ? kAlphaHead : T - nb * kAlphaBlock) : 0;
+    return kAlphaEdge + (nb ? (nb - 1) * kAlphaHead + last : 0) + (n - T);
+}
+
+constexpr uint64_t alpha_chunks(uint64_t n) {
+    if (alpha_whole(n)) return (n + kAlphaChunk - 1) / kAlphaChunk;
+    return kAlphaEdge / kAlphaChunk + alpha_blocks(n) * (kAlphaHead / kAlphaChunk) +
+           (n - alpha_tail_start(n) + kAlphaChunk - 1) / kAlphaChunk;
+}
+constexpr uint64_t alpha_chunk_pos(uint64_t v, uint64_t n) {
+    if (alpha_whole(n) || v < kAlphaEdge / kAlphaChunk) return v * kAlphaChunk;
+    constexpr uint64_t cpb = kAlphaHead / kAlphaChunk;
+    const uint64_t T = alpha_tail_start(n), nb = alpha_blocks(n);
+    v -= kAlphaEdge / kAlphaChunk;
+    if (v < nb * cpb) {
+        const uint64_t pos = (v / cpb + 1) * kAlphaBlock + (v % cpb) * kAlphaChunk;
+        return pos < T ? pos : kAlphaSkip;
+    }
+    return T + (v - nb * cpb) * kAlphaChunk;
+}
+
+}
diff --git a/hpc_suffix_array_amd/csrc/sa_round1.h b/hpc_suffix_array_amd/csrc/sa_round1.h
--- a/hpc_suffix_array_amd/csrc/sa_round1.h
+++ b/hpc_suffix_array_amd/csrc/sa_round1.h
@@ -62,6 +62,7 @@
 }
 constexpr uint64_t kPadMaxN = 1ull << 31;
 constexpr int kUsFlagWord = 12;
+constexpr int kAlphaMissWord = 8;
 
 static uint32_t key1_bits(const BucketSpec& bs) {
     unsigned __int128 dmax = 1;
@@ -204,6 +205,7 @@
     if (bhi <= blo || bhi - blo > (1u << 18)) return set_err(SA_E_INTERNAL, "bucket range [%u, %u)", blo, bhi);
     int rc = onesweep_prepare(c, s);
     if (rc) return rc;
+    uint32_t* const alpha_miss = c->alpha_prove ? c->words + kAlphaMissWord : nullptr;
     SA_HIP(hipMemsetAsync(c->words, 0, 12, s));
     SA_HIP(hipMemsetAsync(c->words + 5, 0, 28, s));
     const bool listed = m * 10 <= n * 3;
@@ -358,7 +360,7 @@
                        (const uint16_t*)c->code, bp.bs, (const uint32_t*)(padded ? pstart : os_base(c)),           \
                        os_tickets(c), c->keys[0], c->vals_alt, g_hi, cursor, m, blo, bhi,                          \
                        padded ? (const uint32_t*)pstart + 1 : nullptr, padded ? c->words + 11 : nullptr, hb, bp.ib, \
-                       stripes)
+                       stripes, alpha_miss)
         if (listed) {
             constexpr int kItemsL = SA_ITEMS_B, kListBlock = SA_LIST_BLOCK;
             const uint64_t tl = (uint64_t)kListBlock * kItemsL;
@@ -380,7 +382,7 @@
                        dim3(kSpBlock), 0, s, d_text, n, (const uint16_t*)c->code, bp.bs,                           \
                        (const uint32_t*)(padded ? pstart : os_base(c)), os_tickets(c), c->keys[0], c->vals_alt, g_hi, \
                        cursor, m, blo, bhi, padded ? (const uint32_t*)pstart + 1 : nullptr,                        \
-                       padded ? c->words + 11 : nullptr, hb, bp.ib, stripes)
+                       padded ? c->words + 11 : nullptr, hb, bp.ib, stripes, alpha_miss)
             if (bp.bs.powR1 * (uint64_t)bp.bs.sigma <= 0xFFFFFFFFull && !(((uint32_t)c->tune >> 28) & 1u))
                 SA_TEXT_NP2(true);
             else
@@ -401,7 +403,7 @@
                                dim3(text_grid(kSpBlock)), dim3(kSpBlock), 0, s, d_text, n, (const uint16_t*)c->code,
                                bp.bs, (const uint32_t*)(padded ? pstart : os_base(c)), os_tickets(c), c->keys[0],
                                c->vals_alt, g_hi, cursor, m, blo, bhi, padded ? (const uint32_t*)pstart + 1 : nullptr,
-                               padded ? c->words + 11 : nullptr, hb, bp.ib, stripes);
+                               padded ? c->words + 11 : nullptr, hb, bp.ib, stripes, alpha_miss);
         } else {
             SA_TEXT_PASS(false, false, kSpBlock, false, false);
         }
@@ -453,14 +455,16 @@
                            dim3(B <= 9 ? kSegBlock : kSpBlock), 0, s, SRC, m, SH,                              \
                            (const uint32_t*)(padded ? pstart : os_base(c)), hbase, c->segw, tk, bp.ib, c->keys_u,      \
                            c->words + 4, padded ? (const uint32_t*)cursor : nullptr,                           \
-                           padded ? (const uint32_t*)dlo : nullptr, stripes, sx);                              \
-    else                                                                                                      \
+                           padded ? (const uint32_t*)dlo : nullptr, stripes, sx,                               \
+                           (const uint32_t*)alpha_miss);                                                       \
+    else                                                                                                     \
         hipLaunchKernelGGL((k_split_seg<S, B, IT, (B <= 9 ? kSegBlock : kSpBlock)>), dim3(grid),                \
                            dim3(B <= 9 ? kSegBlock : kSpBlock), 0, s, SRC, m, SH,                              \
                            (const uint32_t*)(padded ? pstart : os_base(c)), hbase, c->segw, tk, bp.ib, c->keys_u,      \
                            c->words + 4, padded ? (const uint32_t*)cursor : nullptr,                           \
-                           padded ? (const uint32_t*)dlo : nullptr, stripes)
-#define SA_SEG_PASS(B)                                                                                        \
+                           padded ? (const uint32_t*)dlo : nullptr, stripes, SegXq{},                          \
+                           (const uint32_t*)alpha_miss)
+#define SA_SEG_PASS(B)                                                                                       \
     case B:                                                                                                   \
         if (pk8) SA_SEG_LAUNCH(SrcPk8, B, sp, 64u - B, kItemsPk);                                             \
         else SA_SEG_LAUNCH(SrcBucketKeys, B, sb, kLoBits, kItemsB);                                           \
@@ -518,6 +522,11 @@
     SA_HIP(hipMemsetAsync(cnt_u, 0, (2 * nw + 2) * 4, s));
     SA_HIP(hipMemsetAsync(member, 0, (n + 31) / 32 * 4, s));
     SA_HIP(host_sync_event(c->ev[kSyncEv]));
+    if (alpha_miss && c->host_words[kAlphaMissWord]) {
+        SA_TRACE("  bucketed round 1: a byte outside the alphabet sample, again with the exact alphabet");
+        c->alpha_refuted = true;
+        return SA_OK;
+    }
     if (c->host_words[4]) return set_err(SA_E_INTERNAL, "radix look-back did not complete");
     if (padded && c->host_words[11]) {
         SA_TRACE("  bucketed round 1: padded segment overflow, again with exact digit totals");
diff --git a/hpc_suffix_array_amd/csrc/sa_split.h b/hpc_suffix_array_amd/csrc/sa_split.h
--- a/hpc_suffix_array_amd/csrc/sa_split.h
+++ b/hpc_suffix_array_amd/csrc/sa_split.h
@@ -275,7 +275,8 @@
                                                          uint64_t m, uint32_t blo, uint32_t bhi,
                                                          const uint32_t* __restrict__ seg_end = nullptr,
                                                          uint32_t* __restrict__ ovf = nullptr, uint32_t pk_hb = 0,
-                                                         uint32_t pk_ib = 0, uint32_t stripes = 1) {
+                                                         uint32_t pk_ib = 0, uint32_t stripes = 1,
+                                                         uint32_t* __restrict__ alpha_miss = nullptr) {
     constexpr bool NP2 = PK8 && !POW2;
     constexpr int RADIX = kLoRadix;
     constexpr int RWAVES = RADIX / kWave;
@@ -320,9 +321,13 @@
         s_gend[dg] = stripe + 1 == stripes ? hi : sbase + sc;
     }
     cursor += stripe * RADIX;
+    constexpr uint32_t kNoCode = 0xFFu;
+    constexpr uint32_t kStopTicket = 1u << 28;
+    static_assert((0xFFFFFFFFull / TILE + 4096) * SA_TEXT_TPT < kStopTicket, "tickets stay below kStopTicket");
+    const bool prove = alpha_miss != nullptr && b.sigma < 256u;
     if (dg < 256u) {
         const uint32_t cv = code[dg];
-        s_map[dg] = (uint8_t)(cv ? cv - 1u : 0u);
+        s_map[dg] = (uint8_t)(cv ? cv - 1u : prove ? kNoCode : 0u);
     }
     if (dg < (uint32_t)RADIX) s_cnt[dg] = 0;
     constexpr uint32_t TPT = SA_TEXT_TPT;
@@ -391,31 +396,50 @@
 #else
 #define TEXT_STAMP(k)
 #endif
+    auto no_code = [&](uint32_t o, uint32_t& miss) -> uint32_t {
+        if constexpr (IDENT) {
+            return o;
+        } else {
+            const uint32_t hm = ((o & 0x7F7F7F7Fu) + 0x01010101u) & o & 0x80808080u;
+            miss |= hm;
+            return o & ~((hm >> 7) * 0xFFu);
+        }
+    };
+    auto swar = [&](uint32_t rawv, uint32_t& miss) -> uint32_t {
+        const uint32_t o = ((rawv >> 1) ^ (rawv >> 2)) & 0x03030303u;
+        miss |= __builtin_amdgcn_perm(0u, 0x54474341u , o) ^ rawv;
+        return o;
+    };
+    auto map_whole = [&](uint32_t rawv, uint32_t& miss) -> uint32_t {
+        if constexpr (DNA) {
+            return swar(rawv, miss);
+        } else if constexpr (IDENT) {
+            return rawv;
+        } else {
+            return no_code((uint32_t)s_map[rawv & 0xFFu] | ((uint32_t)s_map[(rawv >> 8) & 0xFFu] << 8) |
+                               ((uint32_t)s_map[(rawv >> 16) & 0xFFu] << 16) | ((uint32_t)s_map[rawv >> 24] << 24),
+                           miss);
+        }
+    };
+    auto map_ragged = [&](uint32_t rawv, uint64_t pos, uint32_t& miss) -> uint32_t {
+        uint32_t o = 0;
+#pragma unroll
+        for (int q = 0; q < 4; ++q) o |= (pos + q < n ? (uint32_t)s_map[(rawv >> (8 * q)) & 0xFFu] : 0u) << (8 * q);
+        return no_code(o, miss);
+    };
     auto stage = [&](uint64_t tt) {
         const uint64_t tb = tt * TILE;
+        uint32_t miss = 0;
         const bool whole = (uint32_t)tt < t_whole;
         if constexpr (LD16) {
             if (dg < (uint32_t)NC) {
                 uint32_t o[4];
-#pragma unroll
-                for (int i = 0; i < 4; ++i) {
-                    o[i] = 0;
-                    if (whole) {
-                        if constexpr (DNA)
-                            o[i] = ((raw[i] >> 1) ^ (raw[i] >> 2)) & 0x03030303u;
-                        else if constexpr (IDENT)
-                            o[i] = raw[i];
-                        else
-                            o[i] = (uint32_t)s_map[raw[i] & 0xFFu] | ((uint32_t)s_map[(raw[i] >> 8) & 0xFFu] << 8) |
-                                   ((uint32_t)s_map[(raw[i] >> 16) & 0xFFu] << 16) |
-                                   ((uint32_t)s_map[raw[i] >> 24] << 24);
-                    } else {
-#pragma unroll
-                        for (int q = 0; q < 4; ++q) {
-                            const uint64_t pos = tb + 16ull * dg + 4ull * i + q;
-                            o[i] |= (pos < n ? (uint32_t)s_map[(raw[i] >> (8 * q)) & 0xFFu] : 0u) << (8 * q);
-                        }
-                    }
+                if (whole) {
+#pragma unroll
+                    for (int i = 0; i < 4; ++i) o[i] = map_whole(raw[i], miss);
+                } else {
+#pragma unroll
+                    for (int i = 0; i < 4; ++i) o[i] = map_ragged(raw[i], tb + 16ull * dg + 4ull * i, miss);
                 }
                 if constexpr (DNA) {
                     uint32_t pw = 0;
@@ -433,28 +457,21 @@
         for (int i = 0; i < WPT; ++i) {
             const uint32_t w = dg + i * BLOCK;
             if (w < (uint32_t)NW) {
-                uint32_t o = 0;
-                if (whole) {
-                    if constexpr (DNA)
-                        o = ((raw[i] >> 1) ^ (raw[i] >> 2)) & 0x03030303u;
-                    else if constexpr (IDENT)
-                        o = raw[i];
-                    else
-                        o = (uint32_t)s_map[raw[i] & 0xFFu] | ((uint32_t)s_map[(raw[i] >> 8) & 0xFFu] << 8) |
-                            ((uint32_t)s_map[(raw[i] >> 16) & 0xFFu] << 16) | ((uint32_t)s_map[raw[i] >> 24] << 24);
-                } else {
-#pragma unroll
-                    for (int q = 0; q < 4; ++q) {
-                        const uint64_t pos = tb + 4ull * w + q;
-                        o |= (pos < n ? (uint32_t)s_map[(raw[i] >> (8 * q)) & 0xFFu] : 0u) << (8 * q);
-                    }
-                }
+                const uint32_t o = whole ? map_whole(raw[i], miss) : map_ragged(raw[i], tb + 4ull * w, miss);
                 s_dcw[w] = o;
                 if constexpr (DNA)
                     reinterpret_cast<uint8_t*>(s_pkw)[w] =
                         (uint8_t)(((o & 3u) << 6) | ((o >> 4) & 0x30u) | ((o >> 14) & 0xCu) | (o >> 24));
             }
         }
+        }
+        if (prove && miss) {
+            const uint64_t act = __ballot(1);
+            if (lane == (uint32_t)__ffsll((long long)act) - 1u &&
+                __hip_atomic_load(alpha_miss, __ATOMIC_RELAXED, __HIP_MEMORY_SCOPE_AGENT) == 0u) {
+                atomicOr(alpha_miss, 1u);
+                atomicOr(ticket, kStopTicket);
+            }
         }
     };
     if constexpr (EARLY) {
@@ -892,7 +909,9 @@
                                                         uint32_t* __restrict__ err,
                                                         const uint32_t* __restrict__ seg_cnt = nullptr,
                                                         const uint32_t* __restrict__ dense_lo = nullptr,
-                                                        uint32_t stripes = 1, SegXq xq = SegXq{}) {
+                                                        uint32_t stripes = 1, SegXq xq = SegXq{},
+                                                        const uint32_t* __restrict__ stop = nullptr) {
+    if (stop && *stop) return;
     constexpr int RADIX = 1 << RBITS;
     constexpr int RWAVES = RADIX / kWave;
     constexpr int WTILE = kWave * ITEMS;
diff --git a/include/sa_hip.h b/include/sa_hip.h
--- a/include/sa_hip.h
+++ b/include/sa_hip.h
@@ -63,6 +63,8 @@
 #define SA_DEBUG_FAST32_SMALL 0x2000u
 #define SA_DEBUG_NO_ROUND2_FUSED 0x4000u
 #define SA_DEBUG_LS_ONE_WG 0x8000u
+#define SA_DEBUG_ALPHA_SAMPLE 0x10000u
+#define SA_DEBUG_ALPHA_EXACT 0x20000u
 
 typedef struct {
     int32_t profile;
@@ -99,6 +101,7 @@
     int32_t round1_layout;
     uint64_t round_bytes[SA_MAX_ROUNDS];
     int32_t round1_windows[4];
+    int32_t alphabet_mode;
 } sa_stats;
 
 typedef struct sa_context sa_context;
@@ -236,6 +239,8 @@
 const char* sa_version(void);
 uint64_t sa_host_syncs(void);
 
+int sa_alphabet_sampled(uint64_t pos, uint64_t n);
+
 uint64_t sa_struct_size(int which);
 
 #ifdef __cplusplus
```

New measurement: 111.2 billion (median of 5 runs). 1.01x the previous value.
